# mhalushka/miRge3.0

Measured on NVIDIA B200. Metric: M reads/s trim+collapse+annotate, higher is better.
Workload: dtype u8/int32

## Files before the change

### mirge3.0_b200/csrc/adapter_search.cuh

```cuda
#pragma once
#ifdef ADAPTER_SEARCH_HOST
#include "host_shims.h"
#else
#include "common.cuh"
#endif

#define TRIM_THREADS 128
#define OB 64

struct DevAdapter {
  int where, m, min_overlap, indel_cost, wildcard_ref, k, effective_length;
  int link;
  uint64_t peq[5];
  int n_counts[MIRGE_MAX_ADAPTER_LEN + 1];
  int max_err[MIRGE_MAX_ADAPTER_LEN + 1];
  int acc[MIRGE_MAX_ADAPTER_LEN + 1];
  uint64_t a2;
  int wildcard_read;
  int general;
};
struct DevParams {
  int n_mods, kind[MIRGE_MAX_MODS], a[MIRGE_MAX_MODS], b[MIRGE_MAX_MODS], c[MIRGE_MAX_MODS];
  int n_adapters, times, min_len, umi_mode, umi5, umi3, qia_len, slots;
  int w_mis, w_indel;
  DevAdapter ad[MIRGE_MAX_ADAPTERS];
};
#ifdef ADAPTER_SEARCH_HOST
static DevParams c_p;
#else
__constant__ DevParams c_p;
#endif

static int trim_slots_of(const mirge_trim_params *p) {
  return (p->umi_mode != MIRGE_UMI_QIAGEN && p->count_mode == MIRGE_COUNT_HEAD) ? p->n_mods : 1;
}

#define FILL_FAIL(...)                  \
  do {                                  \
    snprintf(err, err_len, __VA_ARGS__); \
    return MIRGE_ERR_ARG;               \
  } while (0)

static int fill_dev_params(const mirge_trim_params *p, DevParams &d, int &maxm, int &fast_ok, char *err, size_t err_len) {
  if (p->n_mods < 0 || p->n_mods > MIRGE_MAX_MODS) FILL_FAIL("n_mods out of range");
  if (p->n_adapters < 0 || p->n_adapters > MIRGE_MAX_ADAPTERS) FILL_FAIL("n_adapters out of range");
  memset(&d, 0, sizeof(d));
  d.n_mods = p->n_mods;
  for (int i = 0; i < p->n_mods; ++i) {
    if (p->mod_kind[i] < MIRGE_MOD_NEXTSEQ || p->mod_kind[i] > MIRGE_MOD_CUT) FILL_FAIL("unknown modifier kind %d", p->mod_kind[i]);
    d.kind[i] = p->mod_kind[i];
    d.a[i] = p->mod_a[i];
    d.b[i] = p->mod_b[i];
    d.c[i] = p->mod_c[i];
  }
  d.n_adapters = p->n_adapters;
  d.times = p->times;
  d.min_len = p->min_len;
  d.umi_mode = p->umi_mode;
  d.umi5 = p->umi5;
  d.umi3 = p->umi3;
  d.qia_len = p->qia_adapter_len;
  d.slots = trim_slots_of(p);
  if (p->compat != MIRGE_COMPAT_CUTADAPT23 && p->compat != MIRGE_COMPAT_CUTADAPT4) FILL_FAIL("unknown cutadapt compat %d", p->compat);
  d.w_mis = p->compat == MIRGE_COMPAT_CUTADAPT4 ? -1 : 0;
  d.w_indel = p->compat == MIRGE_COMPAT_CUTADAPT4 ? -2 : 0;
  if (p->umi_mode < MIRGE_UMI_NONE || p->umi_mode > MIRGE_UMI_QIAGEN) FILL_FAIL("bad umi_mode");
  if (p->umi_mode != MIRGE_UMI_NONE && (p->umi5 < 0 || p->umi3 < 0)) FILL_FAIL("negative UMI length");
  if (p->umi_mode == MIRGE_UMI_QIAGEN && p->n_adapters < 1) FILL_FAIL("qiagen UMI mode needs an adapter");
  maxm = 0;
  fast_ok = p->n_adapters <= MIRGE_FAST_ADAPTERS;
  for (int a = 0; a < p->n_adapters; ++a) {
    const mirge_adapter *s = &p->adapters[a];
    if (s->m < 1 || s->m > MIRGE_MAX_ADAPTER_LEN) FILL_FAIL("adapter %d length %d unsupported", a, s->m);
    if (s->where < MIRGE_WHERE_BACK || s->where > MIRGE_WHERE_FRONT_NOT_INTERNAL) FILL_FAIL("adapter %d: unknown type", a);
    DevAdapter *o = &d.ad[a];
    o->where = s->where; o->m = s->m; o->min_overlap = s->min_overlap; o->indel_cost = s->indel_cost;
    o->wildcard_ref = s->wildcard_ref; o->k = s->k; o->effective_length = s->effective_length;
    o->link = s->link;
    o->wildcard_read = s->wildcard_read ? 1 : 0;
    o->general = (s->where > MIRGE_WHERE_FRONT || s->wildcard_read) ? 1 : 0;
    if (s->link != 0 && s->link != MIRGE_LINK_BACK_HALF) {
      const int b = (s->link & MIRGE_LINK_INDEX_MASK) - 1;
      if ((s->link & ~(MIRGE_LINK_INDEX_MASK | MIRGE_LINK_FRONT_OPTIONAL | MIRGE_LINK_BACK_OPTIONAL)) || !MIRGE_WHERE_IS_FRONT(s->where) ||
          b <= a || b >= p->n_adapters || MIRGE_WHERE_IS_FRONT(p->adapters[b].where) || p->adapters[b].link != MIRGE_LINK_BACK_HALF)
        FILL_FAIL("adapter %d: a linked pair is a 5' adapter followed by its 3' half", a);
      if (p->umi_mode == MIRGE_UMI_QIAGEN) FILL_FAIL("linked adapters are not supported with qiagen UMIs");
    }
    if (s->link != 0) fast_ok = 0;
    for (int c = 0; c < 4; ++c) {
      uint64_t bits = 0;
      for (int i = 0; i < s->m; ++i)
        if (s->mask[i] & (1 << c)) bits |= 1ull << i;
      o->peq[c] = bits;
    }
    o->peq[4] = 0;
    memcpy(o->n_counts, s->n_counts, sizeof(o->n_counts));
    memcpy(o->max_err, s->max_err, sizeof(o->max_err));
    for (int i = 0; i <= s->m; ++i) {
      const int eff = s->wildcard_ref ? i - s->n_counts[i] : i;
      o->acc[i] = (i >= s->min_overlap && i >= 1 && eff >= 0) ? s->max_err[eff] : -1;
    }
    o->a2 = 0;
    if (!s->wildcard_ref && s->m <= 32)
      for (int i = 0; i < s->m; ++i) {
        const uint64_t code = s->ascii[i] == 'A' ? 0 : s->ascii[i] == 'C' ? 1 : s->ascii[i] == 'G' ? 2 : 3;
        o->a2 |= code << (2 * i);
      }
    if (s->where != MIRGE_WHERE_BACK || s->wildcard_read || s->indel_cost != 1 || s->m > 32 || s->min_overlap < 1 || s->m + 2 * s->k + 3 > 48) fast_ok = 0;
    if (p->compat != MIRGE_COMPAT_CUTADAPT23) fast_ok = 0;
    if (s->m > maxm) maxm = s->m;
  }
  return MIRGE_OK;
}
#undef FILL_FAIL


struct Match { int rstart, rstop, matches, errors; };

#define MS 12
#define MM 0xFFF
__host__ __device__ __forceinline__ uint32_t iupac_set_upper(uint32_t c) {
  c &= 0xDFu;
  switch (c) {
    case 'A': return 1; case 'C': return 2; case 'G': return 4; case 'T': case 'U': return 8;
    case 'R': return 5; case 'Y': return 10; case 'S': return 6; case 'W': return 9; case 'K': return 12; case 'M': return 3;
    case 'B': return 14; case 'D': return 13; case 'H': return 11; case 'V': return 7; case 'N': return 15; default: return 0;
  }
}

template <int MAXM, bool GEN>
__device__ __noinline__ bool locate(const int a, const uint8_t *read, const int n, Match &out) {
  const DevAdapter &ad = c_p.ad[a];
  const int m = ad.m, ic = ad.indel_cost, k = ad.k;
  const bool back = ad.where == 0;
  const int w = ad.where;
  const bool start_in_ref = GEN ? (w == MIRGE_WHERE_FRONT || w == MIRGE_WHERE_FRONT_NOT_INTERNAL) : !back;
  const bool stop_in_ref = GEN ? (w == MIRGE_WHERE_BACK || w == MIRGE_WHERE_BACK_NOT_INTERNAL) : back;
  const bool start_in_query = GEN ? (w != MIRGE_WHERE_PREFIX && w != MIRGE_WHERE_FRONT_NOT_INTERNAL) : true;
  const bool stop_in_query = GEN ? (w != MIRGE_WHERE_SUFFIX && w != MIRGE_WHERE_BACK_NOT_INTERNAL) : true;
  const bool wild_read = GEN && ad.wildcard_read;
  const int max_n = (!GEN || start_in_query) ? n : min(n, m + k);
  const int min_n = (!GEN || stop_in_query) ? 0 : max(0, n - m - k);
  const int w_mis = c_p.w_mis, w_indel = c_p.w_indel;
  const int SB = w_indel ? 2048 : 0;
  const uint64_t p0 = ad.peq[0], p1 = ad.peq[1], p2 = ad.peq[2], p3 = ad.peq[3];
  int cost[MAXM + 1], om[MAXM + 1];
#pragma unroll
  for (int i = 0; i <= MAXM; ++i) {
    if (!GEN) {
      cost[i] = back ? i * ic : 0;
      om[i] = (((back ? 0 : -i) + OB) << MS) + SB + (back ? i * w_indel : 0);
    } else {
      int c, o;
      if (!start_in_ref && !start_in_query) { c = max(i, min_n) * ic; o = 0; }
      else if (start_in_ref && !start_in_query) { c = min_n * ic; o = min(0, min_n - i); }
      else if (!start_in_ref && start_in_query) { c = i * ic; o = max(0, min_n - i); }
      else { c = min(i, min_n) * ic; o = min_n - i; }
      cost[i] = c;
      om[i] = ((o + OB) << MS) + SB + (start_in_ref ? 0 : i * w_indel);
    }
  }
  int best_cost = m + n, best_om = (OB << MS) + (w_indel ? 0 : SB), best_ref_stop = m, best_query_stop = n;
  bool stopped = false;
  for (int j = min_n + 1; j <= max_n; ++j) {
    uint64_t eq;
    if (wild_read) {
      const uint32_t rs = iupac_set_upper(read[j - 1]);
      eq = ((rs & 1u) ? p0 : 0ull) | ((rs & 2u) ? p1 : 0ull) | ((rs & 4u) ? p2 : 0ull) | ((rs & 8u) ? p3 : 0ull);
    } else {
      const uint32_t rc = base_code_upper(read[j - 1]);
      eq = rc == 0 ? p0 : rc == 1 ? p1 : rc == 2 ? p2 : rc == 3 ? p3 : 0ull;
    }
    int dc = cost[0], dom = om[0];
    if (!GEN || start_in_query) om[0] = ((j + OB) << MS) + SB;
    else { cost[0] = j * ic; om[0] = (OB << MS) + SB + j * w_indel; }
    int cm = 0, omm = 0;
#pragma unroll
    for (int i = 1; i <= MAXM; ++i) {
      if (i <= m) {
        int c, o;
        if ((eq >> (i - 1)) & 1ull) {
          c = dc; o = dom + 1;
        } else {
          const int cd = dc + 1, cdel = cost[i] + ic, cins = cost[i - 1] + ic;
          if (cd <= cdel && cd <= cins) { c = cd; o = dom + w_mis; }
          else if (cins <= cdel) { c = cins; o = om[i - 1] + w_indel; }
          else { c = cdel; o = om[i] + w_indel; }
        }
        dc = cost[i]; dom = om[i];
        cost[i] = c; om[i] = o;
        if (i == m) { cm = c; omm = o; }
      }
    }
    if (cm <= k && (!GEN || stop_in_query)) {
      const int origin = (omm >> MS) - OB, mt = omm & MM;
      const int length = m + min(origin, 0);
      int eff = length;
      if (ad.wildcard_ref) eff = (length < m) ? length - (ad.n_counts[m] - ad.n_counts[m - length]) : ad.effective_length;
      const int bm = best_om & MM;
      if (length >= ad.min_overlap && cm <= ad.max_err[eff] && (mt > bm || (mt == bm && cm < best_cost))) {
        best_cost = cm; best_om = omm; best_ref_stop = m; best_query_stop = j;
        if (cm == 0 && mt - SB == m) { stopped = true; break; }
      }
    }
  }
  if (!stopped && (!GEN || max_n == n)) {
    const int first_i = stop_in_ref ? 0 : m;
#pragma unroll
    for (int i = 0; i <= MAXM; ++i) {
      if (i >= first_i && i <= m) {
        const int origin = (om[i] >> MS) - OB, mt = om[i] & MM, c = cost[i];
        const int length = i + min(origin, 0);
        int eff = length;
        if (ad.wildcard_ref) {
          if (length < m) { const int ref_start = origin < 0 ? -origin : 0; eff = length - (ad.n_counts[i] - ad.n_counts[ref_start]); }
          else eff = ad.effective_length;
        }
        const int bm = best_om & MM;
        if (length >= ad.min_overlap && eff >= 0 && c <= ad.max_err[eff] && (mt > bm || (mt == bm && c < best_cost))) {
          best_cost = c; best_om = om[i]; best_ref_stop = i; best_query_stop = n;
        }
      }
    }
  }
  (void)best_ref_stop;
  if (best_cost == m + n) return false;
  const int origin = (best_om >> MS) - OB;
  out.rstart = origin >= 0 ? origin : 0;
  out.rstop = best_query_stop;
  out.matches = (best_om & MM) - SB;
  out.errors = best_cost;
  return true;
}

__device__ __noinline__ bool find_literal(const int a, const uint8_t *read, const int n, Match &out) {
  const DevAdapter &ad = c_p.ad[a];
  const int m = ad.m;
  const uint64_t top = 1ull << (m - 1);
  uint64_t state = 0;
  for (int j = 0; j < n; ++j) {
    const uint32_t rc = base_code_upper(read[j]);
    state = ((state << 1) | 1ull) & (rc < 4u ? ad.peq[rc] : 0ull);
    if (state & top) {
      out.rstart = j + 1 - m;
      out.rstop = j + 1;
      out.matches = m;
      out.errors = 0;
      return true;
    }
  }
  return false;
}

template <int MAXM>
__device__ __forceinline__ bool locate_any(const int a, const uint8_t *read, const int n, Match &out) {
  const DevAdapter &ad = c_p.ad[a];
  if (!ad.general) return locate<MAXM, false>(a, read, n, out);
  if (ad.wildcard_read && !ad.wildcard_ref && ad.where <= MIRGE_WHERE_FRONT && find_literal(a, read, n, out)) return true;
  return locate<MAXM, true>(a, read, n, out);
}

#define RB 48

struct FastCtx {
  const uint32_t *s_eq;
  const uint32_t *ps;
  bool jump_ok;
  int rbase;
};

struct ByteRead {
  const uint8_t *p;
  __device__ __forceinline__ uint32_t eq(const uint32_t *eqt, int j) const { return eqt[p[j]]; }
  struct Cursor {
    const uint8_t *q;
    __device__ __forceinline__ uint32_t next(const uint32_t *eqt) { return eqt[*q++]; }
  };
  __device__ __forceinline__ Cursor cursor() const { return Cursor{p}; }
};
struct PackedRead {
  const uint32_t *ps;
  int base;
  __device__ __forceinline__ uint32_t eq(const uint32_t *eqt, int j) const {
    const int a = base + j;
    return eqt[(ps[(a >> 4) * TRIM_THREADS] >> (2 * (a & 15))) & 3u];
  }
  struct Cursor {
    const uint32_t *row;
    uint32_t w;
    int left;
    __device__ __forceinline__ uint32_t next(const uint32_t *eqt) {
      if (left == 0) {
        row += TRIM_THREADS;
        w = *row;
        left = 16;
      }
      const uint32_t code = w & 3u;
      w >>= 2;
      --left;
      return eqt[code];
    }
  };
  __device__ __forceinline__ Cursor cursor() const {
    const uint32_t *row = ps + (base >> 4) * TRIM_THREADS;
    const int sh = base & 15;
    return Cursor{row, *row >> (2 * sh), 16 - sh};
  }
};

struct ColBuf {
  uint32_t vp[RB], vn[RB];
  int j0;
};

__device__ __forceinline__ int cell_cost(uint32_t vp, uint32_t vn, int r) {
  const uint32_t mask = r >= 32 ? 0xFFFFFFFFu : ((1u << r) - 1u);
  return __popc(vp & mask) - __popc(vn & mask);
}

#define MYERS_STEP(eq, vp, vn, hp_out, hn_out)                    \
  {                                                               \
    const uint32_t xv_ = (eq) | (vn);                             \
    const uint32_t xh_ = ((((eq) & (vp)) + (vp)) ^ (vp)) | (eq);  \
    uint32_t hp_ = (vn) | ~(xh_ | (vp));                          \
    uint32_t hn_ = (vp) & xh_;                                    \
    hp_out = hp_;                                                 \
    hn_out = hn_;                                                 \
    hp_ <<= 1;                                                    \
    hn_ <<= 1;                                                    \
    (vp) = hn_ | ~(xv_ | hp_);                                    \
    (vn) = hp_ & xv_;                                             \
  }

template <class RV>
__device__ __noinline__ void recompute(const uint32_t *eqt, const RV read, int jc, int span, ColBuf &cb) {
  const int j0 = max(0, jc - span);
  uint32_t vp = 0xFFFFFFFFu, vn = 0u;
  cb.j0 = j0;
  cb.vp[0] = vp;
  cb.vn[0] = vn;
  int t = 1;
  for (int j = j0 + 1; j <= jc; ++j, ++t) {
    const uint32_t eq = read.eq(eqt, j - 1);
    uint32_t hp, hn;
    MYERS_STEP(eq, vp, vn, hp, hn)
    cb.vp[t] = vp;
    cb.vn[t] = vn;
  }
}

__device__ __forceinline__ uint64_t read_window(const uint32_t *ps, int a0) {
  const int wi = a0 >> 4, sh = 2 * (a0 & 15);
  const uint32_t w0 = ps[wi * TRIM_THREADS], w1 = ps[(wi + 1) * TRIM_THREADS], w2 = ps[(wi + 2) * TRIM_THREADS];
  const uint32_t lo = __funnelshift_r(w0, w1, sh), hi = __funnelshift_r(w1, w2, sh);
  return ((uint64_t)hi << 32) | lo;
}

template <class RV>
__device__ __noinline__ void traceback(const int a, const uint32_t *eqt, const RV read, const FastCtx &fc, const ColBuf &cb,
                                          int i, int j, int c, int &matches, int &origin) {
  const bool jump = fc.jump_ok && !c_p.ad[a].wildcard_ref;
  const uint64_t a2 = c_p.ad[a].a2;
  int r = i, col = j, cost = c, nonmatch = 0;
  while (r > 0 && cost > 0) {
    if (col == 0) {
      nonmatch += r;
      r = 0;
      break;
    }
    const int delta = col - r;
    if (jump && delta >= 0) {
      uint64_t x = a2 ^ read_window(fc.ps, fc.rbase + delta);
      x = (x | (x >> 1)) & 0x5555555555555555ull;
      if (r < 32) x &= (1ull << (2 * r)) - 1ull;
      if (x == 0) {
        col -= r;
        r = 0;
        break;
      }
      const int t = (64 - __clzll((long long)x) + 1) >> 1;
      col -= r - t;
      r = t;
    } else if ((read.eq(eqt, col - 1) >> (r - 1)) & 1u) {
      --r; --col;
      continue;
    }
    const int t0 = col - cb.j0;
    const uint32_t vp0 = cb.vp[t0], vn0 = cb.vn[t0], vp1 = cb.vp[t0 - 1], vn1 = cb.vn[t0 - 1];
    const int cd = cell_cost(vp1, vn1, r - 1) + 1, cdel = cell_cost(vp1, vn1, r) + 1, cins = cell_cost(vp0, vn0, r - 1) + 1;
    if (cd <= cdel && cd <= cins) { --r; --col; ++nonmatch; cost = cd - 1; }
    else if (cins <= cdel) { --r; ++nonmatch; cost = cins - 1; }
    else { --col; cost = cdel - 1; }
  }
  origin = col - r;
  matches = i - nonmatch;
}

__device__ __forceinline__ bool traceback_cost1(const int a, const FastCtx &fc, int i, int j, int &matches, int &origin) {
  const int delta = j - i;
  if (!fc.jump_ok || c_p.ad[a].wildcard_ref || delta < 0) return false;
  const uint64_t a2 = c_p.ad[a].a2;
  const uint64_t even = 0x5555555555555555ull;
  uint64_t x = a2 ^ read_window(fc.ps, fc.rbase + delta);
  x = (x | (x >> 1)) & even;
  if (i < 32) x &= (1ull << (2 * i)) - 1ull;
  if (x == 0) return false;
  const int t = (64 - __clzll((long long)x) + 1) >> 1;
  const uint64_t below = t - 1 >= 32 ? ~0ull : ((1ull << (2 * (t - 1))) - 1ull);
  if ((x & below) == 0) {
    matches = i - 1;
    origin = delta;
    return true;
  }
  uint64_t y = a2 ^ read_window(fc.ps, fc.rbase + delta + 1);
  y = (y | (y >> 1)) & even & below;
  if (y == 0) {
    matches = i - 1;
    origin = delta + 1;
    return true;
  }
  if (delta < 1) return false;
  const uint64_t upto = t >= 32 ? ~0ull : ((1ull << (2 * t)) - 1ull);
  uint64_t z = a2 ^ read_window(fc.ps, fc.rbase + delta - 1);
  z = (z | (z >> 1)) & even & upto;
  if (z != 0) return false;
  matches = i;
  origin = delta - 1;
  return true;
}

template <class RV>
__device__ __forceinline__ bool all_deletions_possible(const uint32_t *eqt, const RV read, int i, int j, int c) {
  const int o = j - i - c;
  return o >= 0 && (read.eq(eqt, o) & 1u);
}

#define MAY_WIN(u, c, idx) (!have || (u) > b_m || ((u) == b_m && ((c) < b_c || ((c) == b_c && (idx) < b_idx))))
#define TAKE_IF_BETTER(mt, c, org, idx)                                                      \
  if (!have || (mt) > b_m || ((mt) == b_m && ((c) < b_c || ((c) == b_c && (idx) < b_idx)))) { \
    have = true; b_m = (mt); b_c = (c); b_o = (org); b_idx = (idx);                          \
  }
#define Q_COL(v) ((int)((v)&0xFFFFu))
#define Q_COST(v) ((int)(((v) >> 16) & 0xFFu))
#define Q_UB(v, m) ((((v) >> 24) & 1u) ? (m) : (m)-1)
#define Q_CHAIN(v) ((int)((v) >> 25))
#define INS_MASK(eq, vp, hn) (~(eq) & (vp) & ((hn) << 1))
#define CHAIN_LEN(ins, i) (__clz((int)~((ins) << (32 - (i)))))

template <bool DEFER, class RV>
__device__ __forceinline__ int locate_fast(const int a, const RV read, const int n, const FastCtx &fc, Match &out) {
  const unsigned lanes = __activemask();
  const DevAdapter &ad = c_p.ad[a];
  const int m = ad.m;
  const int span = m + 2 * ad.k + 2;
  const uint32_t *eqt = fc.s_eq + a * 256;
  const uint32_t top = 1u << (m - 1);
  const int acc_m = ad.acc[m];
  uint32_t vp = 0xFFFFFFFFu, vn = 0u, eq = 0;
  int score = m;
  bool have = false;
  int b_m = 0, b_c = 0, b_o = 0, b_idx = 0;
  bool stopped = false;
  ColBuf cb;
  uint32_t q0 = 0, q1 = 0, q2 = 0, q3 = 0;
  bool pend = false, pend_ins = false, need_slow = false;
  uint32_t pend_v = 0;

#define FLUSH_QUEUE()                                                                            \
  for (int it_ = 0; it_ < 4; ++it_) {                                                            \
    uint32_t v_ = 0;                                                                             \
    int which_ = -1;                                                                             \
    if (q0 && (!v_ || Q_COST(q0) < Q_COST(v_))) { v_ = q0; which_ = 0; }                         \
    if (q1 && (!v_ || Q_COST(q1) < Q_COST(v_))) { v_ = q1; which_ = 1; }                         \
    if (q2 && (!v_ || Q_COST(q2) < Q_COST(v_))) { v_ = q2; which_ = 2; }                         \
    if (q3 && (!v_ || Q_COST(q3) < Q_COST(v_))) { v_ = q3; which_ = 3; }                         \
    if (which_ < 0) break;                                                                       \
    if (which_ == 0) q0 = 0; else if (which_ == 1) q1 = 0; else if (which_ == 2) q2 = 0; else q3 = 0; \
    const int jc_ = Q_COL(v_), cc_ = Q_COST(v_), t_ = Q_CHAIN(v_);                               \
    const int ir_ = m - t_, cr_ = cc_ - t_;           \
    int ub_ = t_ ? ir_ : Q_UB(v_, m);                                                            \
    if (!t_ && ub_ == m && !all_deletions_possible(eqt, read, m, jc_, cc_)) ub_ = m - 1;        \
    if (MAY_WIN(ub_, cc_, jc_)) {                                                                \
      int mt_, org_;                                                                             \
      if (cr_ == 0) {                                                                            \
        mt_ = ir_; org_ = jc_ - ir_;                                                             \
      } else if (!(cr_ == 1 && traceback_cost1(a, fc, ir_, jc_, mt_, org_))) {                   \
        if (DEFER) { need_slow = true; break; }                                                  \
        recompute(eqt, read, jc_, span, cb);                                                     \
        traceback(a, eqt, read, fc, cb, ir_, jc_, cr_, mt_, org_);                               \
      }                                                                                          \
      TAKE_IF_BETTER(mt_, cc_, org_, jc_)                                                        \
    }                                                                                            \
  }

  uint32_t hp = 0, hn = 0;
  auto cur = read.cursor();
  for (int j = 1; j <= n; ++j) {
    eq = cur.next(eqt);
    MYERS_STEP(eq, vp, vn, hp, hn)
    score += (hp & top) ? 1 : 0;
    score -= (hn & top) ? 1 : 0;
    if (pend) {
      if (!(pend_ins && (eq & top))) {
        if (!q0) q0 = pend_v;
        else if (!q1) q1 = pend_v;
        else if (!q2) q2 = pend_v;
        else if (!q3) q3 = pend_v;
        else {
          FLUSH_QUEUE()
          if (DEFER && need_slow) break;
          q0 = pend_v;
        }
      }
      pend = false;
    }
    if (score <= acc_m && j < n) {
      if (score == 0) {
        have = true; b_m = m; b_c = 0; b_o = j - m; b_idx = j;
        stopped = true;
        break;
      }
      bool is_del = false, is_ins = false;
      const bool is_match = (eq & top) != 0u;
      if (!is_match) {
        const uint32_t hps = hp << 1, hns = hn << 1;
        const bool mis = (((vp & ~hps & ~hns) | (~vp & ~vn & hps)) & top) != 0u;
        if (!mis) {
          if (vp & top) is_ins = true;
          else is_del = true;
        }
      }
      if (!is_del) {
        pend = true;
        pend_ins = is_ins;
        const uint32_t chain = is_ins ? 1u + (uint32_t)CHAIN_LEN(INS_MASK(eq, vp, hn), m - 1) : 0u;
        pend_v = (uint32_t)j | ((uint32_t)score << 16) | (is_match ? (1u << 24) : 0u) | (chain << 25);
      }
    }
  }
  __syncwarp(lanes);
  const unsigned scan_lanes = __ballot_sync(lanes, !stopped && !need_slow);
  if (!stopped && !need_slow) {
    uint32_t rowmask = 0, rowub = 0;
    const uint32_t hps = hp << 1, hns = hn << 1;
    const uint32_t ins = n >= 1 ? INS_MASK(eq, vp, hn) : 0u;
    const uint32_t mis = n >= 1 ? (~eq & ((vp & ~hps & ~hns) | (~vp & ~vn & hps))) : 0u;
    int c = 0;
    for (int i = 1; i <= m; ++i) {
      const uint32_t bit = 1u << (i - 1);
      c += (int)((vp >> (i - 1)) & 1u) - (int)((vn >> (i - 1)) & 1u);
      if (c > ad.acc[i]) continue;
      if (c == 0) {
        const int idx = (i == m) ? n : n + 1 + i;
        TAKE_IF_BETTER(i, 0, n - i, idx)
      } else if (ins & bit) {
        const int t = CHAIN_LEN(ins, i);
        if (ad.acc[i - t] >= c - t) continue;
        rowmask |= bit;
      } else {
        rowmask |= bit;
        if ((eq & bit) || !(mis & bit)) rowub |= bit;
      }
    }
    __syncwarp(scan_lanes);
    FLUSH_QUEUE()
    bool have_cols = false;
    while (rowmask) {
      const int i = 32 - __clz(rowmask);
      const uint32_t bit = 1u << (i - 1);
      rowmask &= ~bit;
      const int ci = cell_cost(vp, vn, i);
      const int idx = (i == m) ? n : n + 1 + i;
      const int t = (ins & bit) ? CHAIN_LEN(ins, i) : 0;
      const int ir = i - t, cr = ci - t;
      int ub = t ? ir : ((rowub & bit) ? i : i - 1);
      if (!t && ub == i && !all_deletions_possible(eqt, read, i, n, ci)) ub = i - 1;
      if (MAY_WIN(ub, ci, idx)) {
        int mt, org;
        if (cr == 0) {
          mt = ir;
          org = n - ir;
        } else if (!(cr == 1 && traceback_cost1(a, fc, ir, n, mt, org))) {
          if (DEFER) { need_slow = true; break; }
          if (!have_cols) {
            recompute(eqt, read, n, span, cb);
            have_cols = true;
          }
          traceback(a, eqt, read, fc, cb, ir, n, cr, mt, org);
        }
        TAKE_IF_BETTER(mt, ci, org, idx)
      }
    }
  }
  if (DEFER && need_slow) return 2;
  if (!have) return 0;
  out.rstart = b_o;
  out.rstop = b_idx <= n ? b_idx : n;
  out.matches = b_m;
  out.errors = b_c;
  return 1;
}


__device__ __forceinline__ int nextseq_trim_index(const uint8_t *seq, const uint8_t *qual, int len, int cutoff, int base) {
  int s = 0, max_qual = 0, max_i = len;
  for (int i = len - 1; i >= 0; --i) {
    int q = (int)qual[i] - base;
    if (seq[i] == 'G') q = cutoff - 1;
    s += cutoff - q;
    if (s < 0) break;
    if (s > max_qual) { max_qual = s; max_i = i; }
  }
  return max_i;
}

__device__ __forceinline__ void quality_trim_index(const uint8_t *qual, int len, int q5, int q3, int base, int &start, int &stop) {
  int s = 0, max_qual = 0;
  start = 0; stop = len;
  for (int i = 0; i < len; ++i) {
    s += q5 - ((int)qual[i] - base);
    if (s < 0) break;
    if (s > max_qual) { max_qual = s; start = i + 1; }
  }
  max_qual = 0; s = 0;
  for (int i = len - 1; i >= 0; --i) {
    s += q3 - ((int)qual[i] - base);
    if (s < 0) break;
    if (s > max_qual) { max_qual = s; stop = i; }
  }
  if (start >= stop) { start = 0; stop = 0; }
}


template <int MAXM, bool FAST, bool DEFER>
__device__ __noinline__ int best_match(const uint8_t *read, int n, Match &best, const FastCtx &fc) {
  int which = -1;
  for (int a = 0; a < c_p.n_adapters; ++a) {
    Match mt;
    const int link = c_p.ad[a].link;
    if (link == MIRGE_LINK_BACK_HALF) continue;
    if (FAST) {
      const int rc = locate_fast<DEFER>(a, ByteRead{read}, n, fc, mt);
      if (rc == 2) return -2;
      if (rc == 0) continue;
    } else if (link != 0) {
      Match f, b;
      const bool have_f = locate_any<MAXM>(a, read, n, f);
      if (!have_f && !(link & MIRGE_LINK_FRONT_OPTIONAL)) continue;
      const int rest = have_f ? f.rstop : 0;
      const bool have_b = locate_any<MAXM>((link & MIRGE_LINK_INDEX_MASK) - 1, read + rest, n - rest, b);
      if (!have_b && (!(link & MIRGE_LINK_BACK_OPTIONAL) || !have_f)) continue;
      mt.rstart = rest;
      mt.rstop = have_b ? rest + b.rstart : n;
      mt.matches = (have_f ? f.matches : 0) + (have_b ? b.matches : 0);
      mt.errors = (have_f ? f.errors : 0) + (have_b ? b.errors : 0);
    } else if (!locate_any<MAXM>(a, read, n, mt)) continue;
    if (which < 0 || mt.matches > best.matches || (mt.matches == best.matches && mt.errors < best.errors)) {
      best = mt;
      which = a;
    }
  }
  return which;
}

template <int MAXM, bool FAST, bool DEFER>
__device__ __noinline__ bool apply_mod(int mi, const uint8_t *seq, const uint8_t *qual, int &start, int &stop, FastCtx &fc) {
  const int len = stop - start;
  switch (c_p.kind[mi]) {
    case MIRGE_MOD_NEXTSEQ:
      stop = start + nextseq_trim_index(seq + start, qual + start, len, c_p.a[mi], c_p.b[mi]);
      break;
    case MIRGE_MOD_QUALITY: {
      int s, e;
      quality_trim_index(qual + start, len, c_p.a[mi], c_p.b[mi], c_p.c[mi], s, e);
      stop = start + e;
      start = start + s;
      break;
    }
    case MIRGE_MOD_ADAPTER:
      for (int t = 0; t < c_p.times; ++t) {
        Match mt;
        fc.rbase = start;
        const int a = best_match<MAXM, FAST, DEFER>(seq + start, stop - start, mt, fc);
        if (a == -2) return true;
        if (a < 0) break;
        if (c_p.ad[a].link != 0) { stop = start + mt.rstop; start = start + mt.rstart; }
        else if (!MIRGE_WHERE_IS_FRONT(c_p.ad[a].where)) stop = start + mt.rstart;
        else start = start + mt.rstop;
      }
      break;
    case MIRGE_MOD_NEND:
      while (start < stop && seq[start] == 'N') ++start;
      while (stop > start && seq[stop - 1] == 'N') --stop;
      break;
    case MIRGE_MOD_CUT: {
      const int c = c_p.a[mi];
      if (c > 0) start += min(c, len);
      else stop = start + max(len + c, 0);
      break;
    }
    default: break;
  }
  return false;
}
```

### mirge3.0_b200/csrc/trim.cu

```cuda
#include "common.cuh"
#include "adapter_search.cuh"

extern "C" int mirge_trim_slots(const mirge_ctx *ctx) {
  if (!ctx || !ctx->params_set) return MIRGE_ERR_ARG;
  return trim_slots_of(&ctx->params);
}

extern "C" int mirge_set_trim_params(mirge_ctx *ctx, const mirge_trim_params *p) {
  if (!ctx || !p) return MIRGE_ERR_ARG;
  DevParams d;
  int maxm = 0, fast_ok = 1;
  const int rc = fill_dev_params(p, d, maxm, fast_ok, ctx->err, sizeof(ctx->err));
  if (rc != MIRGE_OK) return rc;
  MIRGE_CUDA(ctx, cudaSetDevice(ctx->device));
  MIRGE_CUDA(ctx, cudaMemcpyToSymbol(c_p, &d, sizeof(d)));
  ctx->params = *p;
  ctx->params_set = 1;
  ctx->max_adapter_len = maxm;
  ctx->fast_ok = fast_ok;
  int split_ok = fast_ok && p->umi_mode != MIRGE_UMI_QIAGEN, seen_ad = 0;
  for (int i = 0; i < p->n_mods; ++i) {
    if (p->mod_kind[i] == MIRGE_MOD_ADAPTER) seen_ad = 1;
    else if (seen_ad && (p->mod_kind[i] == MIRGE_MOD_NEXTSEQ || p->mod_kind[i] == MIRGE_MOD_QUALITY)) split_ok = 0;
  }
  ctx->split_ok = split_ok && seen_ad;
  return MIRGE_OK;
}

__device__ __forceinline__ void apply_plain_mod(int mi, const uint8_t *seq, const uint8_t *qual, int &start, int &stop) {
  const int len = stop - start;
  const int kind = c_p.kind[mi];
  if (kind == MIRGE_MOD_NEXTSEQ) {
    stop = start + nextseq_trim_index(seq + start, qual + start, len, c_p.a[mi], c_p.b[mi]);
  } else if (kind == MIRGE_MOD_QUALITY) {
    int s, e;
    quality_trim_index(qual + start, len, c_p.a[mi], c_p.b[mi], c_p.c[mi], s, e);
    stop = start + e;
    start = start + s;
  } else if (kind == MIRGE_MOD_NEND) {
    while (start < stop && seq[start] == 'N') ++start;
    while (stop > start && seq[stop - 1] == 'N') --stop;
  } else if (kind == MIRGE_MOD_CUT) {
    const int c = c_p.a[mi];
    if (c > 0) start += min(c, len);
    else stop = start + max(len + c, 0);
  }
}

__device__ __forceinline__ int find_sub(const uint8_t *s, int n, const uint8_t *t, int tl, int from) {
  for (int p = from; p + tl <= n; ++p) {
    int j = 0;
    while (j < tl && s[p + j] == t[j]) ++j;
    if (j == tl) return p;
  }
  return -1;
}

__device__ __forceinline__ uint32_t key_byte(const uint8_t *seq, int start, int l1, int us, int p) {
  return p < l1 ? seq[start + p] : seq[us + p - l1];
}

#define MAX_PACK_WORDS 10
#define PS_ROWS_OF(pw) ((pw) + 3)
__shared__ int s_pack_words;
#define PACK_WORDS s_pack_words
#define PS_ROWS PS_ROWS_OF(s_pack_words)

struct DpEntry {
  uint32_t r;
  uint32_t se;
  uint32_t sl;
  uint32_t pad;
};

struct SlowRec {
  uint32_t r, x, y, z, w, nxt, pad0, pad1;
};
struct SlowSink {
  uint32_t *r_list;
  SlowRec *recs;
  uint64_t cap;
};

__device__ __forceinline__ int first_adapter_mod() {
  int mi_ad = c_p.n_mods;
#pragma unroll 1
  for (int i = c_p.n_mods - 1; i >= 0; --i)
    if (c_p.kind[i] == MIRGE_MOD_ADAPTER) mi_ad = i;
  return mi_ad;
}

__device__ __forceinline__ int exact_find(const uint32_t *ps, uint64_t a2, int m, int start, int stop) {
  const int last = stop - m;
  if (last < start) return -1;
  const uint32_t a_lo = (uint32_t)a2, a_hi = (uint32_t)(a2 >> 32);
  const uint32_t lo_mask = m >= 16 ? 0xFFFFFFFFu : ((1u << (2 * m)) - 1u);
  const uint32_t hi_mask = m <= 16 ? 0u : (m >= 32 ? 0xFFFFFFFFu : ((1u << (2 * (m - 16))) - 1u));
  int wb = start >> 4;
  uint32_t x0 = ps[wb * TRIM_THREADS], x1 = ps[(wb + 1) * TRIM_THREADS], x2 = ps[(wb + 2) * TRIM_THREADS];
#pragma unroll 1
  for (; 16 * wb <= last; ++wb) {
#pragma unroll
    for (int s = 0; s < 16; ++s) {
      const uint32_t lo = s ? __funnelshift_r(x0, x1, 2 * s) : x0;
      if (((lo ^ a_lo) & lo_mask) == 0u) {
        const uint32_t hi = s ? __funnelshift_r(x1, x2, 2 * s) : x1;
        const int p = 16 * wb + s;
        if (((hi ^ a_hi) & hi_mask) == 0u && p >= start && p <= last) return p;
      }
    }
    x0 = x1;
    x1 = x2;
    x2 = (wb + 3 < PS_ROWS) ? ps[(wb + 3) * TRIM_THREADS] : 0u;
  }
  return -1;
}

struct InsList {
  uint2 *off;
  uint64_t cap;
};
#define WORD_BITS 36
#define WORD_MASK ((1ull << WORD_BITS) - 1ull)
#define MAX_LIST_ITEMS (1ull << (64 - WORD_BITS))

__shared__ unsigned int s_stats[2];
__device__ __forceinline__ void init_stats(int pack_words) {
  if (threadIdx.x < 2) s_stats[threadIdx.x] = 0;
  if (threadIdx.x == 0) s_pack_words = pack_words;
}
__device__ __forceinline__ void flush_stats(unsigned long long *ctrl) {
  __syncthreads();
  if (threadIdx.x == 0) {
    if (s_stats[0]) atomicAdd(ctrl + 1, (unsigned long long)s_stats[0]);
    if (s_stats[1]) atomicAdd(ctrl + 4, (unsigned long long)s_stats[1]);
  }
}

template <bool FAST, int PASS>
__device__ __forceinline__ void emit_record(const bool valid, const uint64_t r, const int E, const int slot_lo, const int slot_hi,
                                            const uint8_t *seq, const bool fast_emit, const int *w_start, const int *w_stop,
                                            const int *w_us, const int *w_ue, uint32_t *w_words, const bool to_slow,
                                            ushort4 *__restrict__ win, uint32_t *__restrict__ key_off, uint32_t *__restrict__ keys,
                                            uint64_t keys_cap, unsigned long long *__restrict__ ctrl, const SlowSink ss, const uint4 ls,
                                            const uint32_t nxt, const uint32_t *ps_mine, const InsList il) {
  const int lane = threadIdx.x & 31;
  uint32_t my_words = 0, my_kept = 0, my_alg = 0, same_as_prev = 0, my_items = 0;
  if (valid) {
#pragma unroll 1
    for (int s = slot_lo; s < slot_hi; ++s) {
      if (!w_words[s]) continue;
      ++my_kept;
      if (s > slot_lo && w_words[s - 1] && w_start[s] == w_start[s - 1] && w_stop[s] == w_stop[s - 1] && w_us[s] == w_us[s - 1] &&
          w_ue[s] == w_ue[s - 1]) {
        w_words[s] = w_words[s - 1];
        my_alg += w_words[s];
        same_as_prev |= 1u << s;
        continue;
      }
      if (FAST && fast_emit) {
        w_words[s] = 1u + ((uint32_t)(w_stop[s] - w_start[s] + 15) >> 4);
      } else {
        const int l1 = w_stop[s] - w_start[s], len = l1 + (w_ue[s] - w_us[s]);
        uint32_t nexc = 0;
        for (int p = 0; p < len; ++p) nexc += base_code_exact(key_byte(seq, w_start[s], l1, w_us[s], p)) == 4u;
        w_words[s] = 1u + ((uint32_t)(len + 15) >> 4) + nexc;
      }
      my_words += w_words[s];
      my_alg += w_words[s];
      ++my_items;
    }
  }
  uint32_t inc = my_words | (my_items << 24);
#pragma unroll
  for (int d = 1; d < 32; d <<= 1) {
    const uint32_t t = __shfl_up_sync(0xffffffffu, inc, d);
    if (lane >= d) inc += t;
  }
  const uint32_t both_total = __shfl_sync(0xffffffffu, inc, 31);
  const uint32_t warp_total = both_total & 0xFFFFFFu, warp_items = both_total >> 24;
  const uint32_t item_before = (inc >> 24) - my_items;
  inc &= 0xFFFFFFu;
  const uint32_t kept_warp = __reduce_add_sync(0xffffffffu, my_kept);
  const uint32_t alg_warp = __reduce_add_sync(0xffffffffu, my_alg);
  unsigned long long both = 0;
  if (lane == 0) {
    if (both_total) both = atomicAdd(ctrl + 0, ((unsigned long long)warp_items << WORD_BITS) | (unsigned long long)warp_total);
    if (kept_warp) atomicAdd(&s_stats[0], kept_warp);
    if (alg_warp) atomicAdd(&s_stats[1], alg_warp);
  }
  both = __shfl_sync(0xffffffffu, both, 0);
  const unsigned long long warp_base = both & WORD_MASK, item_base = both >> WORD_BITS;
  const bool overflow = warp_base + warp_total > keys_cap || warp_base + warp_total > 0xFFFFFFF0ull;
  if (overflow && lane == 0 && warp_total) atomicOr(ctrl + 2, 2ull);
  if (PASS == 1) {
    const unsigned sm_ = __ballot_sync(0xffffffffu, to_slow);
    if (sm_) {
      unsigned long long base = 0;
      if (lane == __ffs(sm_) - 1) base = atomicAdd(ctrl + 5, (unsigned long long)__popc(sm_));
      base = __shfl_sync(0xffffffffu, base, __ffs(sm_) - 1);
      if (to_slow) {
        const unsigned long long at = base + __popc(sm_ & ((1u << lane) - 1u));
        if (!ss.recs) {
          ss.r_list[at] = (uint32_t)r;
        } else if (at < ss.cap) {
          SlowRec sr;
          sr.r = (uint32_t)r; sr.x = ls.x; sr.y = ls.y; sr.z = ls.z; sr.w = ls.w; sr.nxt = nxt; sr.pad0 = sr.pad1 = 0;
          *(uint4 *)&ss.recs[at] = *(const uint4 *)&sr;
          *((uint4 *)&ss.recs[at] + 1) = *((const uint4 *)&sr + 1);
        } else {
          atomicOr(ctrl + 2, 8ull);
        }
      }
    }
  }
  if (!valid) return;
  uint32_t off = (uint32_t)warp_base + inc - my_words;
  uint64_t item = item_base + item_before;
#pragma unroll 1
  for (int s = slot_lo; s < slot_hi; ++s) {
    const uint64_t e = r * (uint64_t)E + s;
    if (win) win[e] = make_ushort4((unsigned short)w_start[s], (unsigned short)w_stop[s], (unsigned short)w_us[s], (unsigned short)w_ue[s]);
    if (!w_words[s] || overflow) {
      if (key_off) key_off[e] = 0xFFFFFFFFu;
      continue;
    }
    if ((same_as_prev >> s) & 1u) {
      if (key_off) key_off[e] = off - w_words[s];
      continue;
    }
    if (key_off) key_off[e] = off;
    if (il.off && item < il.cap) {
      const uint32_t run = (uint32_t)__ffs((int)(~(same_as_prev >> (s + 1)) | (1u << (slot_hi - s - 1))));
      il.off[item] = make_uint2(off, run);
      ++item;
    }
    const int l1 = w_stop[s] - w_start[s], len = l1 + (w_ue[s] - w_us[s]);
    const uint32_t npay = (uint32_t)(len + 15) >> 4;
    uint32_t *k = keys + off;
    if (FAST && fast_emit) {
      k[0] = (uint32_t)len;
      const int wi = w_start[s] >> 4;
      const uint32_t bs = 2u * (uint32_t)(w_start[s] & 15);
      uint32_t lo = ps_mine[wi * TRIM_THREADS];
#pragma unroll 1
      for (uint32_t w = 0; w < npay; ++w) {
        const uint32_t hi = ps_mine[(wi + w + 1) * TRIM_THREADS];
        uint32_t v = __funnelshift_r(lo, hi, bs);
        lo = hi;
        const int rem = len - 16 * (int)w;
        if (rem < 16) v &= (1u << (2 * rem)) - 1u;
        k[1 + w] = v;
      }
    } else {
      const uint32_t nexc = w_words[s] - 1u - npay;
      k[0] = (uint32_t)len | (nexc << 16);
      uint32_t word = 0, xi = 0;
      for (int p = 0; p < len; ++p) {
        const uint32_t ch = key_byte(seq, w_start[s], l1, w_us[s], p);
        const uint32_t code = base_code_exact(ch);
        if (code == 4u) k[1 + npay + xi++] = ((uint32_t)p << 8) | ch;
        else word |= code << (2 * (p & 15));
        if ((p & 15) == 15) { k[1 + (p >> 4)] = word; word = 0; }
      }
      if (len & 15) k[1 + (len >> 4)] = word;
    }
    off += w_words[s];
  }
}

#define RECORD_SLOT(mi_)                                                                         \
  if (!qia && (E != 1 || (mi_) == n_mods - 1)) {                                                 \
    const int slot_ = (E == 1) ? 0 : (mi_);                                                      \
    int ln_ = stop - start;                                                                      \
    if (c_p.umi_mode == MIRGE_UMI_FLANKS) ln_ = max(ln_ - c_p.umi5 - c_p.umi3, 0);               \
    w_start[slot_] = start; w_stop[slot_] = stop; w_words[slot_] = ln_ >= c_p.min_len;           \
  }

struct SplitOut {
  DpEntry *entries;
  uint32_t *pk;
  uint64_t cap;
};

template <int MAXM, bool FAST, int PASS, bool SPLIT>
__device__ __forceinline__ void process_record(const bool valid, const uint64_t r, const uint8_t *B, uint64_t nbytes,
                                               const uint32_t *__restrict__ line_start, ushort4 *__restrict__ win,
                                               uint32_t *__restrict__ key_off, uint32_t *__restrict__ keys, uint64_t keys_cap,
                                               unsigned long long *__restrict__ ctrl, const SlowSink ss, FastCtx &fc,
                                               uint32_t *ps_mine, const SplitOut so, const uint4 ls, const uint32_t nxt,
                                               const InsList il) {
  const int lane = threadIdx.x & 31;
  bool is_slow = false;
  const int E = c_p.slots;
  const int n_mods = c_p.n_mods;
  const bool qia = c_p.umi_mode == MIRGE_UMI_QIAGEN;
  int w_start[MIRGE_MAX_MODS], w_stop[MIRGE_MAX_MODS], w_us[MIRGE_MAX_MODS], w_ue[MIRGE_MAX_MODS];
  uint32_t w_words[MIRGE_MAX_MODS];
#pragma unroll 1
  for (int s = 0; s < E; ++s) { w_start[s] = w_stop[s] = w_us[s] = w_ue[s] = 0; w_words[s] = 0; }
  const uint8_t *seq = nullptr, *qual = nullptr;
  uint32_t seq_off = 0;
  bool fast_emit = FAST, good = false;
  int sl = 0, start = 0, stop = 0;
  if (valid) {
    sl = (int)(ls.z - 1 - ls.y);
    int ql = (int)(nxt - 1 - ls.w);
    if (sl > 0 && B[ls.y + sl - 1] == '\r') --sl;
    if (ql > 0 && B[ls.w + ql - 1] == '\r') --ql;
    const bool bad = B[ls.x] != '@' || B[ls.z] != '+' || sl != ql || sl > MIRGE_MAX_READ_LEN;
    if (bad) {
      atomicOr(ctrl + 2, (sl > MIRGE_MAX_READ_LEN && sl == ql) ? 4ull : 1ull);
      atomicMax(ctrl + 3, ~(unsigned long long)r);
    } else {
      good = true;
      seq_off = ls.y;
      seq = B + ls.y;
      qual = B + ls.w;
      stop = sl;
    }
  }
  const unsigned good_lanes = __ballot_sync(0xffffffffu, good);
  if (good && FAST) {
    fast_emit = sl <= 16 * PACK_WORDS;
    if (PASS == 2 && (uint64_t)seq_off + 16 * ((sl + 15) >> 4) + 8 > nbytes) fast_emit = false;
    if (fast_emit) {
      const uint32_t *ap = (const uint32_t *)((uintptr_t)seq & ~(uintptr_t)3);
      const uint32_t bs = ((uint32_t)(uintptr_t)seq & 3u) * 8u;
      const int nwords = (sl + 15) >> 4;
      uint32_t anyexc = 0, prev = ap[0];
      int k = 1;
#pragma unroll 1
      for (int w = 0; w < nwords; ++w) {
        uint32_t word = 0;
#pragma unroll
        for (int q4 = 0; q4 < 4; ++q4) {
          const uint32_t nx = ap[k++];
          const uint32_t quad = __funnelshift_r(prev, nx, bs);
          prev = nx;
          const int nb = sl - (16 * w + 4 * q4);
          uint32_t codes = ((quad >> 1) ^ (quad >> 2)) & 0x03030303u;
          uint32_t sel = codes | (codes >> 4);
          sel = (sel & 0xFFu) | ((sel >> 8) & 0xFF00u);
          uint32_t diff = __byte_perm(0x54474341u, 0u, sel) ^ quad;
          if (nb < 4) {
            const uint32_t tm = nb <= 0 ? 0u : (0xFFFFFFFFu >> (8 * (4 - nb)));
            codes &= tm;
            diff &= tm;
          }
          anyexc |= diff;
          word |= ((codes * 0x01041040u) >> 24) << (8 * q4);
        }
        ps_mine[w * TRIM_THREADS] = word;
      }
#pragma unroll 1
      for (int w = nwords; w < PS_ROWS; ++w) ps_mine[w * TRIM_THREADS] = 0;
      if (anyexc) fast_emit = false;
    }
    fc.jump_ok = fast_emit;
  }

#define RUN_MODS(from_, to_)                                                                     \
  _Pragma("unroll 1") for (int mi = (from_); mi < (to_); ++mi) {                                 \
    if (!is_slow) is_slow = apply_mod<MAXM, FAST, PASS == 1>(mi, seq, qual, start, stop, fc);    \
    __syncwarp(good_lanes);                                                                      \
    RECORD_SLOT(mi)                                                                              \
  }

  int slot_lo = 0, slot_hi = E;
  bool to_slow = false;
  if constexpr (!SPLIT) {
    if (good) { RUN_MODS(0, n_mods) }
  } else {
    const int mi_ad = first_adapter_mod();
    if (good) {
      _Pragma("unroll 1") for (int mi = 0; mi < mi_ad; ++mi) {
        apply_plain_mod(mi, seq, qual, start, stop);
        __syncwarp(good_lanes);
        RECORD_SLOT(mi)
      }
    }
    bool to_dp = false, resolved = false;
    if (good && mi_ad < n_mods) {
      const DevAdapter &ad0 = c_p.ad[0];
      const bool exact_ok = c_p.n_adapters == 1 && c_p.times == 1 && !ad0.wildcard_ref && ad0.acc[ad0.m] >= 0;
      int p = -1;
      if (fc.jump_ok && exact_ok) p = exact_find(ps_mine, ad0.a2, ad0.m, start, stop);
      __syncwarp(good_lanes);
      if (!fc.jump_ok) {
        is_slow = true;
      } else if (p >= 0) {
        stop = p;
        resolved = true;
      } else {
        to_dp = true;
      }
      if (resolved) { RECORD_SLOT(mi_ad) }
    }
    if (good) {
      _Pragma("unroll 1") for (int mi = mi_ad + 1; mi < n_mods; ++mi) {
        if (resolved && !is_slow) {
          const int kind = c_p.kind[mi];
          if (kind == MIRGE_MOD_NEND) {
            while (start < stop && seq[start] == 'N') ++start;
            while (stop > start && seq[stop - 1] == 'N') --stop;
          } else if (kind == MIRGE_MOD_CUT) {
            const int c = c_p.a[mi], len = stop - start;
            if (c > 0) start += min(c, len);
            else stop = start + max(len + c, 0);
          } else {
            is_slow = true;
          }
        }
        __syncwarp(good_lanes);
        if (resolved) { RECORD_SLOT(mi) }
      }
    }
    const unsigned dm = __ballot_sync(0xffffffffu, to_dp);
    if (dm) {
      const int leader = __ffs(dm) - 1;
      unsigned long long base = 0;
      if (lane == leader) base = atomicAdd(ctrl + 6, (unsigned long long)__popc(dm));
      base = __shfl_sync(0xffffffffu, base, leader);
      if (to_dp) {
        const uint64_t e = base + __popc(dm & ((1u << lane) - 1u));
        DpEntry de;
        de.r = (uint32_t)r; de.se = (uint32_t)start | ((uint32_t)stop << 16); de.sl = (uint32_t)sl; de.pad = 0;
        *(uint4 *)(so.entries + e) = *(const uint4 *)&de;
        const int nwords = (sl + 15) >> 4;
#pragma unroll 1
        for (int w = 0; w < nwords; ++w) so.pk[(uint64_t)w * so.cap + e] = ps_mine[w * TRIM_THREADS];
      }
    }
    if (to_dp) slot_hi = (E == 1) ? 0 : mi_ad;
  }
#undef RUN_MODS

  if (good) {
    if (qia) {
      const int tl = stop - start, U = c_p.umi3;
      int us = 0, ue = 0;
      if (tl > 0) {
        const int first = find_sub(seq, sl, seq + start, tl, 0);
        const int after = first + tl;
        const int nx = find_sub(seq, sl, seq + start, tl, after);
        int seg_end = nx < 0 ? sl : nx;
        seg_end = min(seg_end, after + c_p.qia_len + U);
        ue = seg_end;
        us = (U != 0) ? max(seg_end - U, after) : after;
      }
      w_start[0] = start; w_stop[0] = stop; w_us[0] = us; w_ue[0] = ue;
      w_words[0] = (tl >= c_p.min_len) ? 1u : 0u;
      if (ue > us) fast_emit = false;
    }
    if (PASS == 1 && is_slow) {
      slot_hi = slot_lo;
      to_slow = true;
    }
  }
  emit_record<FAST, PASS>(valid, r, E, slot_lo, slot_hi, seq, fast_emit, w_start, w_stop, w_us, w_ue, w_words, to_slow, win, key_off,
                          keys, keys_cap, ctrl, ss, ls, nxt, ps_mine, il);
}

__device__ __noinline__ bool find_lines(const uint8_t *fq, uint64_t n, uint4 &ls, uint32_t &nxt, bool virtual_nl) {
  uint32_t found[4];
  int k = 0;
  for (uint64_t p = ls.x; p < n && k < 4; ++p)
    if (fq[p] == '\n') found[k++] = (uint32_t)p + 1u;
  if (k == 3 && virtual_nl && n > found[2]) found[k++] = (uint32_t)n + 1u;
  if (k < 4) return false;
  ls.y = found[0]; ls.z = found[1]; ls.w = found[2];
  nxt = found[3];
  return true;
}

template <int MAXM, bool FAST, int PASS, bool SPLIT>
__global__ void __launch_bounds__(TRIM_THREADS, (FAST && PASS == 1) ? 7 : 1)
trim_kernel(const uint8_t *__restrict__ fq, uint64_t nbytes, const uint32_t *__restrict__ line_start, uint64_t n_records,
            ushort4 *__restrict__ win, uint32_t *__restrict__ key_off, uint32_t *__restrict__ keys, uint64_t keys_cap,
            unsigned long long *__restrict__ ctrl, uint32_t smem_bytes, uint32_t *__restrict__ d_slow, const SplitOut so,
            const InsList il, const int pack_words, const SlowRec *__restrict__ slow_recs, const uint32_t n_cap) {
  extern __shared__ uint4 smem4[];
  uint8_t *sbuf = (uint8_t *)smem4;
  const int tid = threadIdx.x;
  FastCtx fc;
  fc.s_eq = nullptr; fc.ps = nullptr; fc.jump_ok = false; fc.rbase = 0;
  uint32_t *ps_mine = nullptr;
  init_stats(pack_words);
  if (FAST) {
    uint32_t *eq = (uint32_t *)(sbuf + smem_bytes);
    for (int e = tid; e < c_p.n_adapters * 256; e += TRIM_THREADS) {
      const uint32_t code = base_code_upper((uint32_t)(e & 255));
      eq[e] = code < 4u ? (uint32_t)c_p.ad[e >> 8].peq[code] : 0u;
    }
    fc.s_eq = eq;
    ps_mine = eq + c_p.n_adapters * 256 + tid;
    fc.ps = ps_mine;
  }
  const SlowSink ss{d_slow, nullptr, 0};
  if (PASS == 2) {
    __syncthreads();
    unsigned long long n_slow = ctrl[5];
    if (slow_recs && n_slow > n_cap) n_slow = n_cap;
    const uint64_t first = (uint64_t)blockIdx.x * TRIM_THREADS + (tid & ~31);
    for (uint64_t base = first; base < n_slow; base += (uint64_t)gridDim.x * TRIM_THREADS) {
      const uint64_t idx = base + (tid & 31);
      bool valid = idx < n_slow;
      uint64_t r = 0;
      fc.jump_ok = false;
      uint4 ls = make_uint4(0, 0, 0, 0);
      uint32_t nxt = 0;
      if (valid && slow_recs) {
        const uint4 a = *(const uint4 *)&slow_recs[idx], b = *((const uint4 *)&slow_recs[idx] + 1);
        r = a.x;
        ls = make_uint4(a.y, a.z, a.w, b.x);
        nxt = b.y;
        if (ls.y == 0) valid = find_lines(fq, nbytes, ls, nxt, b.z != 0);
        if (valid && r >= n_cap) {
          atomicOr(ctrl + 2, 16ull);
          valid = false;
        }
        if (valid && line_start) {
          uint32_t *lo = const_cast<uint32_t *>(line_start);
          lo[4 * r] = ls.x; lo[4 * r + 1] = ls.y; lo[4 * r + 2] = ls.z; lo[4 * r + 3] = ls.w; lo[4 * r + 4] = nxt;
        }
      } else if (valid) {
        r = d_slow[idx];
        ls = *(const uint4 *)(line_start + 4 * r);
        nxt = line_start[4 * r + 4];
      }
      process_record<MAXM, FAST, 2, false>(valid, r, fq, nbytes, line_start, win, key_off, keys, keys_cap, ctrl,
                                           ss, fc, ps_mine, so, ls, nxt, il);
      __syncwarp();
    }
    flush_stats(ctrl);
    return;
  }
  const uint64_t r0 = (uint64_t)blockIdx.x * TRIM_THREADS;
  const uint64_t r = r0 + tid;
  const bool valid = r < n_records;
  const uint64_t r_end = min(r0 + (uint64_t)TRIM_THREADS, n_records);
  const uint32_t span_lo = line_start[4 * r0];
  const uint64_t span_hi = min((uint64_t)line_start[4 * r_end], nbytes);
  const uint32_t alo = span_lo & ~15u;
  const bool staged = (span_hi - alo) <= smem_bytes;
  if (FAST && !staged) {
    if (PASS == 1) {
      const unsigned vm = __ballot_sync(0xffffffffu, valid);
      if (vm) {
        const int lane = tid & 31;
        unsigned long long base = 0;
        if (lane == __ffs(vm) - 1) base = atomicAdd(ctrl + 5, (unsigned long long)__popc(vm));
        base = __shfl_sync(0xffffffffu, base, __ffs(vm) - 1);
        if (valid) d_slow[base + __popc(vm & ((1u << lane) - 1u))] = (uint32_t)r;
      }
      return;
    }
    if (tid == 0) atomicOr(ctrl + 2, 8ull);
    return;
  }
  if (staged) {
    for (uint64_t o = (uint64_t)tid * 16; alo + o < span_hi; o += TRIM_THREADS * 16) {
      const uint64_t g = alo + o;
      if (g + 16 <= nbytes) {
        cp_async_16(sbuf + o, fq + g);
      } else {
        for (int b = 0; b < 16 && g + b < nbytes; ++b) sbuf[o + b] = fq[g + b];
      }
    }
    cp_async_wait_all();
  }
  __syncthreads();
  uint4 ls = make_uint4(0, 0, 0, 0);
  uint32_t nxt = 0;
  if (valid) { ls = *(const uint4 *)(line_start + 4 * r); nxt = line_start[4 * r + 4]; }
  const uint8_t *B = staged ? (const uint8_t *)(sbuf - alo) : fq;
  process_record<MAXM, FAST, PASS, SPLIT>(valid, r, B, nbytes, line_start, win, key_off, keys, keys_cap, ctrl, ss, fc, ps_mine, so, ls, nxt, il);
  flush_stats(ctrl);
}

#ifndef DT_TILE
#define DT_TILE 16384
#endif
#define DT_OVH 2048
#define DT_LOAD (DT_TILE + DT_OVH)
#define DT_WORDS (DT_LOAD / 32)
#ifndef DT_NBUF
#define DT_NBUF 2
#endif
#ifndef DT_GROUPS
#define DT_GROUPS 1
#endif
#define DT_CWARPS (DT_GROUPS * TRIM_THREADS / 32)
#define DT_THREADS (32 + DT_GROUPS * TRIM_THREADS)
#define DT_FLAG_AGG (1ull << 62)
#define DT_FLAG_INC (2ull << 62)
#define DT_VAL_MASK ((1ull << 62) - 1ull)
static_assert(DT_TILE % 1024 == 0 && DT_LOAD % 1024 == 0, "the producer scans 1 KB per step");

struct TileMeta {
  unsigned long long before;
  unsigned long long tile_lo;
  uint32_t n_rec;
  uint32_t j0;
  uint32_t nload;
  uint32_t first;
  uint32_t n_nl;
  uint32_t at_end;
};

struct DigestTilesArgs {
  const uint8_t *fq;
  unsigned long long n;
  uint32_t skew;
  uint32_t is_final;
  unsigned long long n_tiles;
  unsigned long long *tile_state;
  uint32_t *line_start;
  uint32_t n_cap;
  ushort4 *win;
  uint32_t *key_off;
  uint32_t *keys;
  unsigned long long keys_cap;
  unsigned long long *ctrl;
  SlowSink ss;
  SplitOut so;
  InsList il;
  int pack_words;
};

__device__ __forceinline__ uint32_t nl_position(const uint32_t *mask, const uint16_t *pref, uint32_t j, uint32_t &w_out) {
  uint32_t lo = 0, hi = DT_WORDS;
  while (hi - lo > 1) {
    const uint32_t mid = (lo + hi) >> 1;
    if (pref[mid] <= j) lo = mid; else hi = mid;
  }
  uint32_t m = mask[lo];
  for (uint32_t k = j - pref[lo]; k; --k) m &= m - 1;
  w_out = lo;
  return 32u * lo + (uint32_t)(__ffs((int)m) - 1);
}
__device__ __forceinline__ uint32_t nl_next(const uint32_t *mask, uint32_t p, uint32_t &w) {
  const uint32_t bit = p & 31u;
  uint32_t m = bit == 31u ? 0u : (mask[w] & (0xFFFFFFFEu << bit));
  while (m == 0u) {
    if (++w >= DT_WORDS) return 0xFFFFFFFFu;
    m = mask[w];
  }
  return 32u * w + (uint32_t)(__ffs((int)m) - 1);
}

__global__ void __launch_bounds__(DT_THREADS, 3) digest_tiles_kernel(const __grid_constant__ DigestTilesArgs A) {
  extern __shared__ uint4 smem4[];
  __shared__ uint64_t bar_full[DT_NBUF], bar_ready[DT_NBUF], bar_empty[DT_NBUF];
  __shared__ TileMeta s_meta[DT_NBUF];
  __shared__ uint32_t s_next[DT_NBUF];
  uint8_t *bufs = (uint8_t *)smem4;
  uint32_t *masks = (uint32_t *)(bufs + DT_NBUF * DT_LOAD);
  uint16_t *prefs = (uint16_t *)(masks + DT_NBUF * DT_WORDS);
  uint32_t *eq = (uint32_t *)(prefs + DT_NBUF * (DT_WORDS + 2));
  uint32_t *ps_base = eq + c_p.n_adapters * 256;
  const int tid = threadIdx.x, lane = tid & 31, warp = tid >> 5;
  unsigned long long *ctrl = A.ctrl;
  init_stats(A.pack_words);
  for (int e = tid; e < c_p.n_adapters * 256; e += DT_THREADS) {
    const uint32_t code = base_code_upper((uint32_t)(e & 255));
    eq[e] = code < 4u ? (uint32_t)c_p.ad[e >> 8].peq[code] : 0u;
  }
  if (tid == 0) {
    for (int b = 0; b < DT_NBUF; ++b) {
      mbar_init(&bar_full[b], 1);
      mbar_init(&bar_ready[b], 1);
      mbar_init(&bar_empty[b], DT_CWARPS);
    }
    asm volatile("fence.mbarrier_init.release.cluster;" ::: "memory");
  }
  __syncthreads();
  const bool virtual_nl = A.is_final && A.n > A.skew && A.fq[A.n - 1] != '\n';

  if (warp == 0) {
    for (uint32_t it = 0;; ++it) {
      const int b = it % DT_NBUF;
      const uint32_t par = (it / DT_NBUF) & 1u;
      if (it >= DT_NBUF) mbar_wait(&bar_empty[b], par ^ 1u);
      unsigned long long t = 0;
      if (lane == 0) t = atomicAdd(ctrl + 11, 1ull);
      t = __shfl_sync(0xffffffffu, t, 0);
      TileMeta &M = s_meta[b];
      if (t >= A.n_tiles) {
        if (lane == 0) {
          M.n_rec = 0xFFFFFFFFu;
          mbar_arrive(&bar_ready[b]);
        }
        break;
      }
      const unsigned long long tile_lo = t * DT_TILE;
      const uint32_t nload = (uint32_t)min((unsigned long long)DT_LOAD, A.n - tile_lo);
      const uint32_t bulk = nload & ~15u;
      uint8_t *buf = bufs + b * DT_LOAD;
      if (lane == 0) {
        if (bulk) {
          mbar_arrive_expect_tx(&bar_full[b], bulk);
          bulk_load(buf, A.fq + tile_lo, bulk, &bar_full[b]);
        } else {
          mbar_arrive(&bar_full[b]);
        }
      }
      if ((uint32_t)lane < nload - bulk) buf[bulk + lane] = A.fq[tile_lo + bulk + lane];
      __syncwarp();
      mbar_wait(&bar_full[b], par);
      uint32_t *mk = masks + b * DT_WORDS;
      uint16_t *pf = prefs + b * (DT_WORDS + 2);
      const uint32_t vpos = (virtual_nl && A.n - tile_lo < DT_LOAD) ? (uint32_t)(A.n - tile_lo) : 0xFFFFFFFFu;
      uint32_t running = 0, tile_total = 0;
#pragma unroll 1
      for (uint32_t w0 = 0; w0 < DT_WORDS; w0 += 32) {
        const uint32_t w = w0 + lane, pos = 32u * w;
        uint32_t m = 0;
        if (pos < nload) {
          const uint4 a = *(const uint4 *)(buf + pos), c = *(const uint4 *)(buf + pos + 16);
          const uint32_t ww[8] = {a.x, a.y, a.z, a.w, c.x, c.y, c.z, c.w};
          m = newline_mask(ww);
          if (pos + 32 > nload) m &= (1u << (nload - pos)) - 1u;
          if (t == 0 && w == 0) m &= ~((1u << A.skew) - 1u);
        }
        if (vpos >= pos && vpos < pos + 32) m |= 1u << (vpos - pos);
        mk[w] = m;
        const uint32_t c = __popc(m);
        uint32_t inc = c;
#pragma unroll
        for (int d = 1; d < 32; d <<= 1) {
          const uint32_t x = __shfl_up_sync(0xffffffffu, inc, d);
          if (lane >= d) inc += x;
        }
        pf[w] = (uint16_t)(running + inc - c);
        running += __shfl_sync(0xffffffffu, inc, 31);
        if (w0 + 32 == DT_TILE / 32) tile_total = running;
      }
      if (lane == 0) pf[DT_WORDS] = (uint16_t)running;
      __syncwarp();
      unsigned long long before = 0;
      if (lane == 0) {
        volatile unsigned long long *st = A.tile_state;
        if (t == 0) {
          st[0] = DT_FLAG_INC | (unsigned long long)tile_total;
        } else {
          st[t] = DT_FLAG_AGG | (unsigned long long)tile_total;
          __threadfence();
          unsigned long long p = t;
          while (true) {
            --p;
            unsigned long long v;
            while (((v = st[p]) >> 62) == 0ull) {}
            before += v & DT_VAL_MASK;
            if ((v >> 62) == 2ull) break;
          }
          st[t] = DT_FLAG_INC | (before + tile_total);
        }
        __threadfence();
        if (tile_total) atomicAdd(ctrl + 9, (unsigned long long)tile_total);
      }
      before = __shfl_sync(0xffffffffu, before, 0);
      const uint32_t j0 = (3u - (uint32_t)(before & 3ull)) & 3u;
      const uint32_t n_rec = tile_total > j0 ? (tile_total - j0 + 3u) / 4u : 0u;
      if (lane == 0) {
        if (n_rec) {
          uint32_t wq;
          const uint32_t pe = nl_position(mk, pf, j0 + 4u * (n_rec - 1u), wq);
          atomicMax(ctrl + 10, tile_lo + pe + 1ull);
        }
        M.before = before; M.tile_lo = tile_lo; M.n_rec = n_rec; M.j0 = j0; M.nload = nload; M.first = t == 0 ? 1u : 0u;
        M.n_nl = running; M.at_end = tile_lo + nload >= A.n ? 1u : 0u;
        s_next[b] = 0;
        __threadfence_block();
        mbar_arrive(&bar_ready[b]);
      }
      __syncwarp();
    }
  } else {
    const int ctid = tid - 32, group = ctid / TRIM_THREADS;
    uint32_t *ps_mine = ps_base + group * PS_ROWS_OF(A.pack_words) * TRIM_THREADS + (ctid & (TRIM_THREADS - 1));
    FastCtx fc;
    fc.s_eq = eq; fc.ps = ps_mine; fc.jump_ok = false; fc.rbase = 0;
    for (uint32_t it = 0;; ++it) {
      const int b = it % DT_NBUF;
      const uint32_t par = (it / DT_NBUF) & 1u;
      mbar_wait(&bar_ready[b], par);
      const TileMeta M = s_meta[b];
      if (M.n_rec == 0xFFFFFFFFu) break;
      const uint32_t *mk = masks + b * DT_WORDS;
      const uint16_t *pf = prefs + b * (DT_WORDS + 2);
      const uint8_t *B = bufs + b * DT_LOAD - M.tile_lo;
      const uint32_t total = M.n_rec + M.first;
      while (true) {
        uint32_t c = 0;
        if (lane == 0) c = atomicAdd(&s_next[b], 32u);
        c = __shfl_sync(0xffffffffu, c, 0);
        if (c >= total) break;
        const uint32_t q = c + lane;
        bool valid = q < total, far = false;
        uint64_t r = 0;
        uint4 ls = make_uint4(0, 0, 0, 0);
        uint32_t nxt = 0;
        if (valid) {
          uint32_t p, w = 0;
          if (M.first && q == 0) {
            ls.x = A.skew;
            p = 0xFFFFFFFFu;
          } else {
            const uint32_t j = M.j0 + 4u * (q - M.first);
            p = nl_position(mk, pf, j, w);
            ls.x = (uint32_t)M.tile_lo + p + 1u;
            r = (M.before + j + 1ull) >> 2;
          }
          uint32_t e[4];
          bool all = true;
#pragma unroll
          for (int k = 0; k < 4; ++k) {
            if (all) {
              if (p == 0xFFFFFFFFu && k == 0) {
                p = M.n_nl ? nl_position(mk, pf, 0u, w) : 0xFFFFFFFFu;
              } else {
                p = nl_next(mk, p, w);
              }
              all = p != 0xFFFFFFFFu;
              e[k] = (uint32_t)M.tile_lo + p + 1u;
            }
          }
          if (all) {
            ls.y = e[0]; ls.z = e[1]; ls.w = e[2];
            nxt = e[3];
          } else if (M.at_end) {
            valid = false;
          } else {
            far = true;
            valid = false;
          }
          if ((valid || far) && r >= A.n_cap) {
            atomicOr(ctrl + 2, 16ull);
            valid = far = false;
          }
          if (valid && A.line_start) {
            *(uint4 *)(A.line_start + 4 * r) = ls;
            A.line_start[4 * r + 4] = nxt;
          }
        }
        const unsigned fm = __ballot_sync(0xffffffffu, far);
        if (fm) {
          unsigned long long fb = 0;
          if (lane == __ffs(fm) - 1) fb = atomicAdd(ctrl + 5, (unsigned long long)__popc(fm));
          fb = __shfl_sync(0xffffffffu, fb, __ffs(fm) - 1);
          if (far) {
            const unsigned long long at = fb + __popc(fm & ((1u << lane) - 1u));
            if (at < A.ss.cap) {
              SlowRec sr;
              sr.r = (uint32_t)r; sr.x = ls.x; sr.y = 0; sr.z = 0; sr.w = 0; sr.nxt = 0; sr.pad0 = virtual_nl ? 1u : 0u; sr.pad1 = 0;
              *(uint4 *)&A.ss.recs[at] = *(const uint4 *)&sr;
              *((uint4 *)&A.ss.recs[at] + 1) = *((const uint4 *)&sr + 1);
            } else {
              atomicOr(ctrl + 2, 8ull);
            }
          }
        }
        process_record<32, true, 1, true>(valid, r, B, A.n, nullptr, A.win, A.key_off, A.keys, A.keys_cap, ctrl, A.ss, fc, ps_mine,
                                          A.so, ls, nxt, A.il);
        __syncwarp();
      }
      __syncwarp();
      if (lane == 0) mbar_arrive(&bar_empty[b]);
    }
  }
  flush_stats(ctrl);
}

template <bool FIRST>
__global__ void __launch_bounds__(TRIM_THREADS, FIRST ? 7 : 4)
trim_dp_kernel(const DpEntry *__restrict__ entries, const uint32_t *__restrict__ pk, uint64_t cap, uint32_t *__restrict__ redo,
               ushort4 *__restrict__ win, uint32_t *__restrict__ key_off, uint32_t *__restrict__ keys, uint64_t keys_cap,
               unsigned long long *__restrict__ ctrl, const InsList il, const int pack_words) {
  extern __shared__ uint4 smem4[];
  uint32_t *eq = (uint32_t *)smem4;
  uint32_t *ps_base = eq + c_p.n_adapters * 256;
  DpEntry *s_ent = (DpEntry *)(ps_base + PS_ROWS_OF(pack_words) * TRIM_THREADS);
  uint32_t *s_hist = (uint32_t *)(s_ent + TRIM_THREADS);
  uint16_t *s_order = (uint16_t *)(s_hist + TRIM_THREADS);
  const int tid = threadIdx.x, lane = tid & 31;
  const unsigned long long n_items = FIRST ? ctrl[6] : ctrl[7];
  const uint64_t base = (uint64_t)blockIdx.x * TRIM_THREADS;
  if (base >= n_items) return;
  init_stats(pack_words);
  for (int e = tid; e < c_p.n_adapters * 4; e += TRIM_THREADS) eq[(e >> 2) * 256 + (e & 3)] = (uint32_t)c_p.ad[e >> 2].peq[e & 3];
  const int n_here = (int)min((unsigned long long)TRIM_THREADS, n_items - base);
  uint32_t my_e = 0;
  int bin = TRIM_THREADS - 1;
  if (tid < n_here) {
    my_e = FIRST ? (uint32_t)(base + tid) : redo[base + tid];
    const uint4 v = *(const uint4 *)(entries + my_e);
    DpEntry de = *(const DpEntry *)&v;
    de.pad = my_e;
    s_ent[tid] = de;
    const int wl = (int)(de.se >> 16) - (int)(de.se & 0xFFFFu);
    bin = TRIM_THREADS - 1 - min(wl, TRIM_THREADS - 1);
  }
  s_hist[tid] = 0;
  __syncthreads();
  if (tid < n_here) atomicAdd(&s_hist[bin], 1u);
  __syncthreads();
  if (tid < 32) {
    uint32_t h[TRIM_THREADS / 32], sum = 0;
#pragma unroll
    for (int q = 0; q < TRIM_THREADS / 32; ++q) { h[q] = s_hist[(TRIM_THREADS / 32) * tid + q]; sum += h[q]; }
    uint32_t incl = sum;
#pragma unroll
    for (int d = 1; d < 32; d <<= 1) {
      const uint32_t x = __shfl_up_sync(0xffffffffu, incl, d);
      if (lane >= d) incl += x;
    }
    uint32_t run = incl - sum;
#pragma unroll
    for (int q = 0; q < TRIM_THREADS / 32; ++q) { s_hist[(TRIM_THREADS / 32) * tid + q] = run; run += h[q]; }
  }
  __syncthreads();
  if (tid < n_here) s_order[atomicAdd(&s_hist[bin], 1u)] = (uint16_t)tid;
  __syncthreads();
  const bool valid = tid < n_here;
  const int E = c_p.slots, n_mods = c_p.n_mods;
  const bool qia = false;
  int w_start[MIRGE_MAX_MODS], w_stop[MIRGE_MAX_MODS], w_us[MIRGE_MAX_MODS], w_ue[MIRGE_MAX_MODS];
  uint32_t w_words[MIRGE_MAX_MODS];
#pragma unroll 1
  for (int s = 0; s < E; ++s) { w_start[s] = w_stop[s] = w_us[s] = w_ue[s] = 0; w_words[s] = 0; }
  uint32_t *ps_mine = ps_base + tid;
  const int mi_ad = first_adapter_mod();
  uint64_t r = 0;
  bool need_redo = false;
  int slot_lo = (E == 1) ? 0 : mi_ad, slot_hi = E;
  uint32_t ent_id = 0;
  if (valid) {
    const DpEntry de = s_ent[s_order[tid]];
    r = de.r;
    ent_id = de.pad;
    int start = (int)(de.se & 0xFFFFu), stop = (int)(de.se >> 16);
    const int nwords = ((int)de.sl + 15) >> 4;
#pragma unroll 1
    for (int w = 0; w < PS_ROWS_OF(pack_words); ++w) {
      if (w < nwords) cp_async_4(ps_mine + w * TRIM_THREADS, pk + (uint64_t)w * cap + ent_id);
      else ps_mine[w * TRIM_THREADS] = 0u;
    }
    cp_async_wait_all();
    FastCtx fc;
    fc.s_eq = eq; fc.ps = ps_mine; fc.jump_ok = true; fc.rbase = 0;
#pragma unroll 1
    for (int mi = mi_ad; mi < n_mods && !need_redo; ++mi) {
      const int kind = c_p.kind[mi];
      if (kind == MIRGE_MOD_ADAPTER) {
#pragma unroll 1
        for (int t = 0; t < c_p.times; ++t) {
          fc.rbase = start;
          const PackedRead rv{ps_mine, start};
          const int n = stop - start;
          Match best;
          int which = -1;
#pragma unroll 1
          for (int a = 0; a < c_p.n_adapters; ++a) {
            Match mt;
            const int rc = locate_fast<FIRST>(a, rv, n, fc, mt);
            if (rc == 2) { need_redo = true; break; }
            if (rc == 0) continue;
            if (which < 0 || mt.matches > best.matches || (mt.matches == best.matches && mt.errors < best.errors)) { best = mt; which = a; }
          }
          if (need_redo || which < 0) break;
          stop = start + best.rstart;
        }
      } else if (kind == MIRGE_MOD_CUT) {
        const int c = c_p.a[mi], len = stop - start;
        if (c > 0) start += min(c, len);
        else stop = start + max(len + c, 0);
      }
      if (!need_redo) { RECORD_SLOT(mi) }
    }
  }
  if (FIRST) {
    const unsigned rm = __ballot_sync(0xffffffffu, need_redo);
    if (rm) {
      const int leader = __ffs(rm) - 1;
      unsigned long long b2 = 0;
      if (lane == leader) b2 = atomicAdd(ctrl + 7, (unsigned long long)__popc(rm));
      b2 = __shfl_sync(0xffffffffu, b2, leader);
      if (need_redo) redo[b2 + __popc(rm & ((1u << lane) - 1u))] = ent_id;
    }
    if (need_redo) slot_hi = slot_lo;
  }
  emit_record<true, 0>(valid, r, E, slot_lo, slot_hi, nullptr, true, w_start, w_stop, w_us, w_ue, w_words, false, win, key_off, keys, keys_cap,
                       ctrl, SlowSink{nullptr, nullptr, 0}, make_uint4(0, 0, 0, 0), 0u, ps_mine, il);
  flush_stats(ctrl);
}

static uint64_t align16(uint64_t x) { return (x + 15) & ~15ull; }
extern "C" uint64_t mirge_trim_scratch_bytes(uint64_t n_records) {
  const uint64_t n = n_records ? n_records : 1;
  return 2 * align16(4 * n) + align16(sizeof(DpEntry) * n) + align16(4ull * MAX_PACK_WORDS * n) + 64;
}

extern "C" int mirge_trim(mirge_ctx *ctx, const uint8_t *d_fastq, uint64_t nbytes, const uint32_t *d_line_start, uint64_t n_records,
                          uint16_t *d_win, uint32_t *d_key_off, uint32_t *d_keys, uint64_t keys_capacity_words,
                          uint64_t *d_trim_ctrl, void *d_scratch, uint64_t *d_ins, uint64_t ins_capacity, void *stream_) {
  if (!ctx) return MIRGE_ERR_ARG;
  if (!ctx->params_set) MIRGE_FAIL(ctx, MIRGE_ERR_ARG, "trim: mirge_set_trim_params has not been called");
  if (n_records == 0) return MIRGE_OK;
  if (!d_fastq || !d_line_start || !d_keys || !d_trim_ctrl) MIRGE_FAIL(ctx, MIRGE_ERR_ARG, "trim: null buffer");
  if (!d_win != !d_key_off) MIRGE_FAIL(ctx, MIRGE_ERR_ARG, "trim: d_win and d_key_off go together");
  if (!d_key_off && !d_ins) MIRGE_FAIL(ctx, MIRGE_ERR_ARG, "trim: neither per-slot outputs nor an insert list requested");
  if (d_ins && (ins_capacity == 0 || ((uintptr_t)d_ins & 7))) MIRGE_FAIL(ctx, MIRGE_ERR_ARG, "trim: bad insert list");
  if (n_records * (uint64_t)trim_slots_of(&ctx->params) >= MAX_LIST_ITEMS)
    MIRGE_FAIL(ctx, MIRGE_ERR_ARG, "trim: more than 2^28 emission slots in one batch (use smaller batches)");
  if (((uintptr_t)d_line_start & 15) || ((uintptr_t)d_win & 7) || ((uintptr_t)d_scratch & 15))
    MIRGE_FAIL(ctx, MIRGE_ERR_ARG, "trim: misaligned buffer");
  const InsList il{(uint2 *)d_ins, d_ins ? ins_capacity : 0};
  if (n_records >= 0x80000000ull) MIRGE_FAIL(ctx, MIRGE_ERR_ARG, "trim: more than 2^31 records in one batch");
  {
    const uint32_t skew = (uint32_t)((uintptr_t)d_fastq & 15);
    d_fastq -= skew;
    nbytes += skew;
  }
  cudaStream_t stream = (cudaStream_t)stream_;
  MIRGE_CUDA(ctx, cudaSetDevice(ctx->device));
  const uint64_t avg = (nbytes + n_records - 1) / n_records;
  const bool fast = ctx->fast_ok && ctx->trim_mode != 1;
  const bool split = fast && ctx->split_ok && ctx->trim_mode == 0;
  uint64_t want = fast ? avg * TRIM_THREADS * 33 / 32 + 512 : avg * TRIM_THREADS * 5 / 4 + 64;
  want = (want + 255) & ~255ull;
  if (want < 4096) want = 4096;
  if (want > 96 * 1024) want = 96 * 1024;
  const uint32_t smem = (uint32_t)want;
  const unsigned grid = (unsigned)((n_records + TRIM_THREADS - 1) / TRIM_THREADS);
  unsigned long long *ctrl = (unsigned long long *)d_trim_ctrl;
  ushort4 *win = (ushort4 *)d_win;
  SplitOut so;
  so.entries = nullptr; so.pk = nullptr; so.cap = 0;
  if (fast) {
    if (!d_scratch) MIRGE_FAIL(ctx, MIRGE_ERR_ARG, "trim: scratch of mirge_trim_scratch_bytes(n_records) bytes is required");
    uint8_t *sc = (uint8_t *)d_scratch;
    uint32_t *d_slow = (uint32_t *)sc;
    uint32_t *d_redo = (uint32_t *)(sc + align16(4 * n_records));
    so.entries = (DpEntry *)(sc + 2 * align16(4 * n_records));
    so.pk = (uint32_t *)(sc + 2 * align16(4 * n_records) + align16(sizeof(DpEntry) * n_records));
    so.cap = n_records;
    const int pack_words = avg <= 2 * 112 + 40 ? 8 : MAX_PACK_WORDS;
    const size_t extra = (size_t)ctx->params.n_adapters * 1024 + (size_t)PS_ROWS_OF(pack_words) * TRIM_THREADS * 4;
    if (split) {
      MIRGE_CUDA(ctx, cudaFuncSetAttribute(trim_kernel<32, true, 1, true>, cudaFuncAttributeMaxDynamicSharedMemorySize, 200 * 1024));
      trim_kernel<32, true, 1, true><<<grid, TRIM_THREADS, smem + extra, stream>>>(d_fastq, nbytes, d_line_start, n_records, win, d_key_off,
                                                                                 d_keys, keys_capacity_words, ctrl, smem, d_slow, so, il, pack_words, nullptr, 0u);
      MIRGE_LAUNCH_CHECK(ctx, "trim_kernel(stage 1)");
      const size_t dp_smem = extra + (size_t)TRIM_THREADS * (sizeof(DpEntry) + 4 + 2);
      trim_dp_kernel<true><<<grid, TRIM_THREADS, dp_smem, stream>>>(so.entries, so.pk, so.cap, d_redo, win, d_key_off, d_keys,
                                                                    keys_capacity_words, ctrl, il, pack_words);
      MIRGE_LAUNCH_CHECK(ctx, "trim_dp_kernel(stage 2)");
      trim_dp_kernel<false><<<grid, TRIM_THREADS, dp_smem, stream>>>(so.entries, so.pk, so.cap, d_redo, win, d_key_off, d_keys,
                                                                     keys_capacity_words, ctrl, il, pack_words);
      MIRGE_LAUNCH_CHECK(ctx, "trim_dp_kernel(stage 3)");
    } else {
      MIRGE_CUDA(ctx, cudaFuncSetAttribute(trim_kernel<32, true, 1, false>, cudaFuncAttributeMaxDynamicSharedMemorySize, 200 * 1024));
      trim_kernel<32, true, 1, false><<<grid, TRIM_THREADS, smem + extra, stream>>>(d_fastq, nbytes, d_line_start, n_records, win,
                                                                                  d_key_off, d_keys, keys_capacity_words, ctrl, smem,
                                                                                  d_slow, so, il, pack_words, nullptr, 0u);
      MIRGE_LAUNCH_CHECK(ctx, "trim_kernel(pass 1)");
    }
    unsigned grid2 = split ? grid / 4 + 1 : grid / 16 + 1;
    if (grid2 > (unsigned)ctx->sm_count * (split ? 64u : 8u)) grid2 = (unsigned)ctx->sm_count * (split ? 64u : 8u);
    trim_kernel<32, true, 2, false><<<grid2, TRIM_THREADS, extra, stream>>>(d_fastq, nbytes, d_line_start, n_records, win, d_key_off,
                                                                          d_keys, keys_capacity_words, ctrl, 0u, d_slow, so, il, pack_words, nullptr, 0u);
  } else if (ctx->max_adapter_len <= 32) {
    MIRGE_CUDA(ctx, cudaFuncSetAttribute(trim_kernel<32, false, 0, false>, cudaFuncAttributeMaxDynamicSharedMemorySize, 96 * 1024));
    trim_kernel<32, false, 0, false><<<grid, TRIM_THREADS, smem, stream>>>(d_fastq, nbytes, d_line_start, n_records, win, d_key_off,
                                                                           d_keys, keys_capacity_words, ctrl, smem, nullptr, so, il, 8, nullptr, 0u);
  } else {
    MIRGE_CUDA(ctx, cudaFuncSetAttribute(trim_kernel<64, false, 0, false>, cudaFuncAttributeMaxDynamicSharedMemorySize, 96 * 1024));
    trim_kernel<64, false, 0, false><<<grid, TRIM_THREADS, smem, stream>>>(d_fastq, nbytes, d_line_start, n_records, win, d_key_off,
                                                                           d_keys, keys_capacity_words, ctrl, smem, nullptr, so, il, 8, nullptr, 0u);
  }
  MIRGE_LAUNCH_CHECK(ctx, "trim_kernel");
  return MIRGE_OK;
}

static uint64_t dt_tiles(uint64_t nbytes) { return (nbytes + 16) / DT_TILE + 1; }
static uint64_t dt_slow_cap(uint64_t n_cap) { return n_cap; }

extern "C" int mirge_digest_fused_ok(const mirge_ctx *ctx) {
  if (!ctx || !ctx->params_set) return 0;
  return ctx->fast_ok && ctx->split_ok && ctx->trim_mode == 0;
}

extern "C" uint64_t mirge_digest_scratch_bytes(uint64_t nbytes, uint64_t n_cap) {
  const uint64_t n = n_cap ? n_cap : 1;
  return align16(8 * dt_tiles(nbytes)) + align16(sizeof(SlowRec) * dt_slow_cap(n)) + align16(4 * n) + align16(sizeof(DpEntry) * n) +
         align16(4ull * MAX_PACK_WORDS * n) + 64;
}

extern "C" int mirge_digest_tiles(mirge_ctx *ctx, const uint8_t *d_fastq, uint64_t nbytes, int is_final, uint64_t n_cap,
                                  uint32_t *d_line_start, uint16_t *d_win, uint32_t *d_key_off, uint32_t *d_keys,
                                  uint64_t keys_capacity_words, uint64_t *d_trim_ctrl, void *d_scratch, uint64_t *d_ins,
                                  uint64_t ins_capacity, void *stream_) {
  if (!ctx) return MIRGE_ERR_ARG;
  if (!ctx->params_set) MIRGE_FAIL(ctx, MIRGE_ERR_ARG, "digest: mirge_set_trim_params has not been called");
  if (!mirge_digest_fused_ok(ctx)) MIRGE_FAIL(ctx, MIRGE_ERR_ARG, "digest: the fused path needs 3' adapters of <= 32 nt with indels (use mirge_trim)");
  if (nbytes == 0) return MIRGE_OK;
  if (!d_fastq || !d_keys || !d_trim_ctrl || !d_scratch || n_cap == 0) MIRGE_FAIL(ctx, MIRGE_ERR_ARG, "digest: null buffer");
  if (nbytes > 0xFFFFFF00ull) MIRGE_FAIL(ctx, MIRGE_ERR_ARG, "digest: batch larger than 4 GiB - 256");
  if (!d_win != !d_key_off) MIRGE_FAIL(ctx, MIRGE_ERR_ARG, "digest: d_win and d_key_off go together");
  if (!d_key_off && !d_ins) MIRGE_FAIL(ctx, MIRGE_ERR_ARG, "digest: neither per-slot outputs nor an insert list requested");
  if (d_ins && (ins_capacity < n_cap * (uint64_t)trim_slots_of(&ctx->params) || ((uintptr_t)d_ins & 7)))
    MIRGE_FAIL(ctx, MIRGE_ERR_ARG, "digest: bad insert list");
  if (((uintptr_t)d_line_start & 15) || ((uintptr_t)d_win & 7) || ((uintptr_t)d_scratch & 15)) MIRGE_FAIL(ctx, MIRGE_ERR_ARG, "digest: misaligned buffer");
  if (n_cap >= 0x80000000ull || n_cap * (uint64_t)trim_slots_of(&ctx->params) >= MAX_LIST_ITEMS)
    MIRGE_FAIL(ctx, MIRGE_ERR_ARG, "digest: more than 2^28 emission slots in one batch (use smaller batches)");
  cudaStream_t stream = (cudaStream_t)stream_;
  MIRGE_CUDA(ctx, cudaSetDevice(ctx->device));
  const uint32_t skew = (uint32_t)((uintptr_t)d_fastq & 15);
  DigestTilesArgs A;
  A.fq = d_fastq - skew;
  A.n = nbytes + skew;
  A.skew = skew;
  A.is_final = is_final ? 1u : 0u;
  A.n_tiles = A.n / DT_TILE + 1;
  uint8_t *sc = (uint8_t *)d_scratch;
  A.tile_state = (unsigned long long *)sc;
  sc += align16(8 * dt_tiles(nbytes));
  A.ss.r_list = nullptr;
  A.ss.recs = (SlowRec *)sc;
  A.ss.cap = dt_slow_cap(n_cap);
  sc += align16(sizeof(SlowRec) * A.ss.cap);
  uint32_t *d_redo = (uint32_t *)sc;
  sc += align16(4 * n_cap);
  A.so.entries = (DpEntry *)sc;
  sc += align16(sizeof(DpEntry) * n_cap);
  A.so.pk = (uint32_t *)sc;
  A.so.cap = n_cap;
  A.line_start = d_line_start;
  A.n_cap = (uint32_t)n_cap;
  A.win = (ushort4 *)d_win;
  A.key_off = d_key_off;
  A.keys = d_keys;
  A.keys_cap = keys_capacity_words;
  A.ctrl = (unsigned long long *)d_trim_ctrl;
  A.il = InsList{(uint2 *)d_ins, d_ins ? ins_capacity : 0};
  const uint64_t avg = (nbytes + n_cap - 1) / n_cap;
  A.pack_words = avg <= 2 * 112 + 40 ? 8 : MAX_PACK_WORDS;
  MIRGE_CUDA(ctx, cudaMemsetAsync(A.tile_state, 0, 8 * A.n_tiles, stream));
  const size_t rows = (size_t)PS_ROWS_OF(A.pack_words) * TRIM_THREADS * 4;
  const size_t dt_smem = (size_t)DT_NBUF * DT_LOAD + (size_t)DT_NBUF * DT_WORDS * 4 + (size_t)DT_NBUF * (DT_WORDS + 2) * 2 +
                         (size_t)ctx->params.n_adapters * 1024 + DT_GROUPS * rows;
  MIRGE_CUDA(ctx, cudaFuncSetAttribute(digest_tiles_kernel, cudaFuncAttributeMaxDynamicSharedMemorySize, 200 * 1024));
  int per_sm = 0;
  MIRGE_CUDA(ctx, cudaOccupancyMaxActiveBlocksPerMultiprocessor(&per_sm, digest_tiles_kernel, DT_THREADS, dt_smem));
  if (per_sm < 1) MIRGE_FAIL(ctx, MIRGE_ERR_CUDA, "digest: the fused kernel does not fit an SM");
  uint64_t grid = (uint64_t)ctx->sm_count * per_sm;
  if (grid > A.n_tiles) grid = A.n_tiles;
  digest_tiles_kernel<<<(unsigned)grid, DT_THREADS, dt_smem, stream>>>(A);
  MIRGE_LAUNCH_CHECK(ctx, "digest_tiles_kernel");
  const unsigned lgrid = (unsigned)((n_cap + TRIM_THREADS - 1) / TRIM_THREADS);
  const size_t extra = (size_t)ctx->params.n_adapters * 1024 + rows;
  const size_t dp_smem = extra + (size_t)TRIM_THREADS * (sizeof(DpEntry) + 4 + 2);
  trim_dp_kernel<true><<<lgrid, TRIM_THREADS, dp_smem, stream>>>(A.so.entries, A.so.pk, A.so.cap, d_redo, A.win, d_key_off, d_keys,
                                                                 keys_capacity_words, A.ctrl, A.il, A.pack_words);
  MIRGE_LAUNCH_CHECK(ctx, "trim_dp_kernel(stage 2)");
  trim_dp_kernel<false><<<lgrid, TRIM_THREADS, dp_smem, stream>>>(A.so.entries, A.so.pk, A.so.cap, d_redo, A.win, d_key_off, d_keys,
                                                                  keys_capacity_words, A.ctrl, A.il, A.pack_words);
  MIRGE_LAUNCH_CHECK(ctx, "trim_dp_kernel(stage 3)");
  unsigned grid2 = lgrid / 4 + 1;
  if (grid2 > (unsigned)ctx->sm_count * 64u) grid2 = (unsigned)ctx->sm_count * 64u;
  trim_kernel<32, true, 2, false><<<grid2, TRIM_THREADS, extra, stream>>>(A.fq, A.n, d_line_start, n_cap, A.win, d_key_off, d_keys,
                                                                        keys_capacity_words, A.ctrl, 0u, nullptr, A.so, A.il,
                                                                        A.pack_words, A.ss.recs, (uint32_t)n_cap);
  MIRGE_LAUNCH_CHECK(ctx, "trim_kernel(whole-pipeline pass)");
  return MIRGE_OK;
}

extern "C" int mirge_trim_mode(mirge_ctx *ctx, int mode) {
  if (!ctx || mode < 0 || mode > 2) return MIRGE_ERR_ARG;
  ctx->trim_mode = mode;
  return MIRGE_OK;
}
```

Before: 1234.

## Resume deferred DP reads from saved state and move per-read scratch to shared memory

The DP trimming kernel now saves the Myers search state (bit vectors, queue, best match, loop position) into a per-entry resume record when stage 2 defers a read. Stage 3 can then continue from that point instead of rescanning the read from the start. Per-thread slot arrays and the traceback column buffer move from local memory to shared memory. The kernels become grid-stride loops launched through a helper. The intent is to cut redundant recomputation and local-memory spills, at the cost of extra global scratch, more shared memory per block that may lower occupancy, and a more complex control flow.

New measurement: 1206, median of 6. -2.2%, worse.

```diff
diff --git a/mirge3.0_b200/csrc/adapter_search.cuh b/mirge3.0_b200/csrc/adapter_search.cuh
--- a/mirge3.0_b200/csrc/adapter_search.cuh
+++ b/mirge3.0_b200/csrc/adapter_search.cuh
@@ -267,6 +267,7 @@
   const uint32_t *ps;
   bool jump_ok;
   int rbase;
+  uint32_t *cols;
 };
 
 struct ByteRead {
@@ -309,8 +310,25 @@
 };
 
 struct ColBuf {
-  uint32_t vp[RB], vn[RB];
+  uint32_t vp_[RB], vn_[RB];
   int j0;
+  using Ref = ColBuf &;
+  __device__ __forceinline__ void bind(const FastCtx &) {}
+  __device__ __forceinline__ uint32_t vp(int t) const { return vp_[t]; }
+  __device__ __forceinline__ uint32_t vn(int t) const { return vn_[t]; }
+  __device__ __forceinline__ void set(int t, uint32_t vp, uint32_t vn) { vp_[t] = vp; vn_[t] = vn; }
+};
+struct SharedColBuf {
+  uint32_t *p;
+  int j0;
+  using Ref = SharedColBuf;
+  __device__ __forceinline__ void bind(const FastCtx &fc) { p = fc.cols; }
+  __device__ __forceinline__ uint32_t vp(int t) const { return p[2 * t * TRIM_THREADS]; }
+  __device__ __forceinline__ uint32_t vn(int t) const { return p[(2 * t + 1) * TRIM_THREADS]; }
+  __device__ __forceinline__ void set(int t, uint32_t vp, uint32_t vn) {
+    p[2 * t * TRIM_THREADS] = vp;
+    p[(2 * t + 1) * TRIM_THREADS] = vn;
+  }
 };
 
 __device__ __forceinline__ int cell_cost(uint32_t vp, uint32_t vn, int r) {
@@ -332,20 +350,16 @@
     (vn) = hp_ & xv_;                                             \
   }
 
-template <class RV>
-__device__ __noinline__ void recompute(const uint32_t *eqt, const RV read, int jc, int span, ColBuf &cb) {
-  const int j0 = max(0, jc - span);
+template <class RV, class CBR>
+__device__ __noinline__ void recompute(const uint32_t *eqt, const RV read, int jc, CBR cb) {
   uint32_t vp = 0xFFFFFFFFu, vn = 0u;
-  cb.j0 = j0;
-  cb.vp[0] = vp;
-  cb.vn[0] = vn;
+  cb.set(0, vp, vn);
   int t = 1;
-  for (int j = j0 + 1; j <= jc; ++j, ++t) {
+  for (int j = cb.j0 + 1; j <= jc; ++j, ++t) {
     const uint32_t eq = read.eq(eqt, j - 1);
     uint32_t hp, hn;
     MYERS_STEP(eq, vp, vn, hp, hn)
-    cb.vp[t] = vp;
-    cb.vn[t] = vn;
+    cb.set(t, vp, vn);
   }
 }
 
@@ -356,9 +370,10 @@
   return ((uint64_t)hi << 32) | lo;
 }
 
-template <class RV>
-__device__ __noinline__ void traceback(const int a, const uint32_t *eqt, const RV read, const FastCtx &fc, const ColBuf &cb,
-                                          int i, int j, int c, int &matches, int &origin) {
+struct TraceOut { int matches, origin; };
+template <class RV, class CBR>
+__device__ __noinline__ TraceOut traceback(const int a, const uint32_t *eqt, const RV read, const FastCtx fc, const CBR cb,
+                                           int i, int j, int c) {
   const bool jump = fc.jump_ok && !c_p.ad[a].wildcard_ref;
   const uint64_t a2 = c_p.ad[a].a2;
   int r = i, col = j, cost = c, nonmatch = 0;
@@ -386,14 +401,13 @@
       continue;
     }
     const int t0 = col - cb.j0;
-    const uint32_t vp0 = cb.vp[t0], vn0 = cb.vn[t0], vp1 = cb.vp[t0 - 1], vn1 = cb.vn[t0 - 1];
+    const uint32_t vp0 = cb.vp(t0), vn0 = cb.vn(t0), vp1 = cb.vp(t0 - 1), vn1 = cb.vn(t0 - 1);
     const int cd = cell_cost(vp1, vn1, r - 1) + 1, cdel = cell_cost(vp1, vn1, r) + 1, cins = cell_cost(vp0, vn0, r - 1) + 1;
     if (cd <= cdel && cd <= cins) { --r; --col; ++nonmatch; cost = cd - 1; }
     else if (cins <= cdel) { --r; ++nonmatch; cost = cins - 1; }
     else { --col; cost = cdel - 1; }
   }
-  origin = col - r;
-  matches = i - nonmatch;
+  return TraceOut{i - nonmatch, col - r};
 }
 
 __device__ __forceinline__ bool traceback_cost1(const int a, const FastCtx &fc, int i, int j, int &matches, int &origin) {
@@ -447,8 +461,15 @@
 #define INS_MASK(eq, vp, hn) (~(eq) & (vp) & ((hn) << 1))
 #define CHAIN_LEN(ins, i) (__clz((int)~((ins) << (32 - (i)))))
 
-template <bool DEFER, class RV>
-__device__ __forceinline__ int locate_fast(const int a, const RV read, const int n, const FastCtx &fc, Match &out) {
+struct FastResume {
+  uint32_t st;
+  uint32_t vp, vn, hp, hn, eq;
+  uint32_t q0, q1, q2, q3;
+  uint32_t bo;
+};
+template <bool DEFER, class RV, class CB = ColBuf>
+__device__ __forceinline__ int locate_fast(const int a, const RV read, const int n, const FastCtx &fc, Match &out,
+                                           FastResume *rs = nullptr) {
   const unsigned lanes = __activemask();
   const DevAdapter &ad = c_p.ad[a];
   const int m = ad.m;
@@ -460,8 +481,9 @@
   int score = m;
   bool have = false;
   int b_m = 0, b_c = 0, b_o = 0, b_idx = 0;
-  bool stopped = false;
-  ColBuf cb;
+  bool stopped = false, in_tail = false;
+  CB cb;
+  cb.bind(fc);
   uint32_t q0 = 0, q1 = 0, q2 = 0, q3 = 0;
   bool pend = false, pend_ins = false, need_slow = false;
   uint32_t pend_v = 0;
@@ -475,7 +497,6 @@
     if (q2 && (!v_ || Q_COST(q2) < Q_COST(v_))) { v_ = q2; which_ = 2; }                         \
     if (q3 && (!v_ || Q_COST(q3) < Q_COST(v_))) { v_ = q3; which_ = 3; }                         \
     if (which_ < 0) break;                                                                       \
-    if (which_ == 0) q0 = 0; else if (which_ == 1) q1 = 0; else if (which_ == 2) q2 = 0; else q3 = 0; \
     const int jc_ = Q_COL(v_), cc_ = Q_COST(v_), t_ = Q_CHAIN(v_);                               \
     const int ir_ = m - t_, cr_ = cc_ - t_;           \
     int ub_ = t_ ? ir_ : Q_UB(v_, m);                                                            \
@@ -486,16 +507,27 @@
         mt_ = ir_; org_ = jc_ - ir_;                                                             \
       } else if (!(cr_ == 1 && traceback_cost1(a, fc, ir_, jc_, mt_, org_))) {                   \
         if (DEFER) { need_slow = true; break; }                                                  \
-        recompute(eqt, read, jc_, span, cb);                                                     \
-        traceback(a, eqt, read, fc, cb, ir_, jc_, cr_, mt_, org_);                               \
+        cb.j0 = max(0, jc_ - span);                                                              \
+        recompute<RV, typename CB::Ref>(eqt, read, jc_, cb);                                     \
+        const TraceOut to_ = traceback<RV, typename CB::Ref>(a, eqt, read, fc, cb, ir_, jc_, cr_); \
+        mt_ = to_.matches; org_ = to_.origin;                                                    \
       }                                                                                          \
       TAKE_IF_BETTER(mt_, cc_, org_, jc_)                                                        \
     }                                                                                            \
+    if (which_ == 0) q0 = 0; else if (which_ == 1) q1 = 0; else if (which_ == 2) q2 = 0; else q3 = 0; \
   }
 
   uint32_t hp = 0, hn = 0;
+  const bool resume = !DEFER && rs && (rs->st & 1u);
+  if (resume) {
+    const FastResume s = *rs;
+    have = (s.st >> 1) & 1u; b_m = (int)((s.st >> 8) & 0xFFu); b_c = (int)((s.st >> 16) & 0xFFu);
+    b_o = (int)(s.bo & 0xFFFFu); b_idx = (int)(s.bo >> 16);
+    vp = s.vp; vn = s.vn; hp = s.hp; hn = s.hn; eq = s.eq;
+    q0 = s.q0; q1 = s.q1; q2 = s.q2; q3 = s.q3;
+  }
   auto cur = read.cursor();
-  for (int j = 1; j <= n; ++j) {
+  for (int j = 1; j <= (resume ? 0 : n); ++j) {
     eq = cur.next(eqt);
     MYERS_STEP(eq, vp, vn, hp, hn)
     score += (hp & top) ? 1 : 0;
@@ -541,6 +573,7 @@
   __syncwarp(lanes);
   const unsigned scan_lanes = __ballot_sync(lanes, !stopped && !need_slow);
   if (!stopped && !need_slow) {
+    in_tail = true;
     uint32_t rowmask = 0, rowub = 0;
     const uint32_t hps = hp << 1, hns = hn << 1;
     const uint32_t ins = n >= 1 ? INS_MASK(eq, vp, hn) : 0u;
@@ -583,16 +616,31 @@
         } else if (!(cr == 1 && traceback_cost1(a, fc, ir, n, mt, org))) {
           if (DEFER) { need_slow = true; break; }
           if (!have_cols) {
-            recompute(eqt, read, n, span, cb);
+            cb.j0 = max(0, n - span);
+            recompute<RV, typename CB::Ref>(eqt, read, n, cb);
             have_cols = true;
           }
-          traceback(a, eqt, read, fc, cb, ir, n, cr, mt, org);
+          const TraceOut to = traceback<RV, typename CB::Ref>(a, eqt, read, fc, cb, ir, n, cr);
+          mt = to.matches;
+          org = to.origin;
         }
         TAKE_IF_BETTER(mt, ci, org, idx)
       }
     }
   }
-  if (DEFER && need_slow) return 2;
+  if (DEFER && need_slow) {
+    if (rs && in_tail) {
+      FastResume s;
+      s.st = 1u | (have ? 2u : 0u) | ((uint32_t)b_m << 8) | ((uint32_t)b_c << 16);
+      s.vp = vp; s.vn = vn; s.hp = hp; s.hn = hn; s.eq = eq;
+      s.q0 = q0; s.q1 = q1; s.q2 = q2; s.q3 = q3;
+      s.bo = (uint32_t)b_o | ((uint32_t)b_idx << 16);
+      *rs = s;
+    } else if (rs) {
+      rs->st = 0u;
+    }
+    return 2;
+  }
   if (!have) return 0;
   out.rstart = b_o;
   out.rstop = b_idx <= n ? b_idx : n;
diff --git a/mirge3.0_b200/csrc/trim.cu b/mirge3.0_b200/csrc/trim.cu
--- a/mirge3.0_b200/csrc/trim.cu
+++ b/mirge3.0_b200/csrc/trim.cu
@@ -873,11 +873,23 @@
   flush_stats(ctrl);
 }
 
+struct DpResume {
+  uint32_t pos;
+  uint32_t t;
+  uint32_t se;
+  uint32_t best;
+  FastResume fast;
+  uint32_t pad;
+};
+static_assert(sizeof(DpResume) == 64, "DpResume is four 16-byte words");
+
+#define DP_SLOT_STRIDE(E) ((E) | 1)
+
 template <bool FIRST>
 __global__ void __launch_bounds__(TRIM_THREADS, FIRST ? 7 : 4)
 trim_dp_kernel(const DpEntry *__restrict__ entries, const uint32_t *__restrict__ pk, uint64_t cap, uint32_t *__restrict__ redo,
-               ushort4 *__restrict__ win, uint32_t *__restrict__ key_off, uint32_t *__restrict__ keys, uint64_t keys_cap,
-               unsigned long long *__restrict__ ctrl, const InsList il, const int pack_words) {
+               DpResume *__restrict__ rsm, ushort4 *__restrict__ win, uint32_t *__restrict__ key_off, uint32_t *__restrict__ keys,
+               uint64_t keys_cap, unsigned long long *__restrict__ ctrl, const InsList il, const int pack_words) {
   extern __shared__ uint4 smem4[];
   uint32_t *eq = (uint32_t *)smem4;
   uint32_t *ps_base = eq + c_p.n_adapters * 256;
@@ -885,121 +897,182 @@
   uint32_t *s_hist = (uint32_t *)(s_ent + TRIM_THREADS);
   uint16_t *s_order = (uint16_t *)(s_hist + TRIM_THREADS);
   const int tid = threadIdx.x, lane = tid & 31;
+  const int E = c_p.slots, n_mods = c_p.n_mods, ws = DP_SLOT_STRIDE(E);
+  uint32_t *s_slots = (uint32_t *)(s_order + TRIM_THREADS);
+  int *w_start = (int *)s_slots + tid * ws, *w_stop = (int *)s_slots + (TRIM_THREADS + tid) * ws;
+  uint32_t *w_words = s_slots + (2 * TRIM_THREADS + tid) * ws;
+  const int *w_zero = (const int *)s_slots + 3 * TRIM_THREADS * ws;
+  uint32_t *cols = s_slots + (3 * TRIM_THREADS + 1) * ws + tid;
   const unsigned long long n_items = FIRST ? ctrl[6] : ctrl[7];
-  const uint64_t base = (uint64_t)blockIdx.x * TRIM_THREADS;
-  if (base >= n_items) return;
+  if ((uint64_t)blockIdx.x * TRIM_THREADS >= n_items) return;
   init_stats(pack_words);
   for (int e = tid; e < c_p.n_adapters * 4; e += TRIM_THREADS) eq[(e >> 2) * 256 + (e & 3)] = (uint32_t)c_p.ad[e >> 2].peq[e & 3];
-  const int n_here = (int)min((unsigned long long)TRIM_THREADS, n_items - base);
-  uint32_t my_e = 0;
-  int bin = TRIM_THREADS - 1;
-  if (tid < n_here) {
-    my_e = FIRST ? (uint32_t)(base + tid) : redo[base + tid];
-    const uint4 v = *(const uint4 *)(entries + my_e);
-    DpEntry de = *(const DpEntry *)&v;
-    de.pad = my_e;
-    s_ent[tid] = de;
-    const int wl = (int)(de.se >> 16) - (int)(de.se & 0xFFFFu);
-    bin = TRIM_THREADS - 1 - min(wl, TRIM_THREADS - 1);
-  }
-  s_hist[tid] = 0;
-  __syncthreads();
-  if (tid < n_here) atomicAdd(&s_hist[bin], 1u);
-  __syncthreads();
-  if (tid < 32) {
-    uint32_t h[TRIM_THREADS / 32], sum = 0;
+  for (int s = tid; s < ws; s += TRIM_THREADS) ((int *)w_zero)[s] = 0;
+  for (uint64_t base = (uint64_t)blockIdx.x * TRIM_THREADS; base < n_items; base += (uint64_t)gridDim.x * TRIM_THREADS) {
+    const int n_here = (int)min((unsigned long long)TRIM_THREADS, n_items - base);
+    int bin = TRIM_THREADS - 1;
+    if (tid < n_here) {
+      const uint32_t my_e = FIRST ? (uint32_t)(base + tid) : redo[base + tid];
+      const uint4 v = *(const uint4 *)(entries + my_e);
+      DpEntry de = *(const DpEntry *)&v;
+      de.pad = my_e;
+      s_ent[tid] = de;
+      const int wl = (int)(de.se >> 16) - (int)(de.se & 0xFFFFu);
+      bin = TRIM_THREADS - 1 - min(wl, TRIM_THREADS - 1);
+    }
+    s_hist[tid] = 0;
+    __syncthreads();
+    if (tid < n_here) atomicAdd(&s_hist[bin], 1u);
+    __syncthreads();
+    if (tid < 32) {
+      uint32_t h[TRIM_THREADS / 32], sum = 0;
 #pragma unroll
-    for (int q = 0; q < TRIM_THREADS / 32; ++q) { h[q] = s_hist[(TRIM_THREADS / 32) * tid + q]; sum += h[q]; }
-    uint32_t incl = sum;
+      for (int q = 0; q < TRIM_THREADS / 32; ++q) { h[q] = s_hist[(TRIM_THREADS / 32) * tid + q]; sum += h[q]; }
+      uint32_t incl = sum;
 #pragma unroll
-    for (int d = 1; d < 32; d <<= 1) {
-      const uint32_t x = __shfl_up_sync(0xffffffffu, incl, d);
-      if (lane >= d) incl += x;
-    }
-    uint32_t run = incl - sum;
+      for (int d = 1; d < 32; d <<= 1) {
+        const uint32_t x = __shfl_up_sync(0xffffffffu, incl, d);
+        if (lane >= d) incl += x;
+      }
+      uint32_t run = incl - sum;
 #pragma unroll
-    for (int q = 0; q < TRIM_THREADS / 32; ++q) { s_hist[(TRIM_THREADS / 32) * tid + q] = run; run += h[q]; }
-  }
-  __syncthreads();
-  if (tid < n_here) s_order[atomicAdd(&s_hist[bin], 1u)] = (uint16_t)tid;
-  __syncthreads();
-  const bool valid = tid < n_here;
-  const int E = c_p.slots, n_mods = c_p.n_mods;
-  const bool qia = false;
-  int w_start[MIRGE_MAX_MODS], w_stop[MIRGE_MAX_MODS], w_us[MIRGE_MAX_MODS], w_ue[MIRGE_MAX_MODS];
-  uint32_t w_words[MIRGE_MAX_MODS];
-#pragma unroll 1
-  for (int s = 0; s < E; ++s) { w_start[s] = w_stop[s] = w_us[s] = w_ue[s] = 0; w_words[s] = 0; }
-  uint32_t *ps_mine = ps_base + tid;
-  const int mi_ad = first_adapter_mod();
-  uint64_t r = 0;
-  bool need_redo = false;
-  int slot_lo = (E == 1) ? 0 : mi_ad, slot_hi = E;
-  uint32_t ent_id = 0;
-  if (valid) {
-    const DpEntry de = s_ent[s_order[tid]];
-    r = de.r;
-    ent_id = de.pad;
-    int start = (int)(de.se & 0xFFFFu), stop = (int)(de.se >> 16);
-    const int nwords = ((int)de.sl + 15) >> 4;
-#pragma unroll 1
-    for (int w = 0; w < PS_ROWS_OF(pack_words); ++w) {
-      if (w < nwords) cp_async_4(ps_mine + w * TRIM_THREADS, pk + (uint64_t)w * cap + ent_id);
-      else ps_mine[w * TRIM_THREADS] = 0u;
-    }
-    cp_async_wait_all();
-    FastCtx fc;
-    fc.s_eq = eq; fc.ps = ps_mine; fc.jump_ok = true; fc.rbase = 0;
-#pragma unroll 1
-    for (int mi = mi_ad; mi < n_mods && !need_redo; ++mi) {
-      const int kind = c_p.kind[mi];
-      if (kind == MIRGE_MOD_ADAPTER) {
-#pragma unroll 1
-        for (int t = 0; t < c_p.times; ++t) {
-          fc.rbase = start;
-          const PackedRead rv{ps_mine, start};
-          const int n = stop - start;
-          Match best;
-          int which = -1;
-#pragma unroll 1
-          for (int a = 0; a < c_p.n_adapters; ++a) {
-            Match mt;
-            const int rc = locate_fast<FIRST>(a, rv, n, fc, mt);
-            if (rc == 2) { need_redo = true; break; }
-            if (rc == 0) continue;
-            if (which < 0 || mt.matches > best.matches || (mt.matches == best.matches && mt.errors < best.errors)) { best = mt; which = a; }
+      for (int q = 0; q < TRIM_THREADS / 32; ++q) { s_hist[(TRIM_THREADS / 32) * tid + q] = run; run += h[q]; }
+    }
+    __syncthreads();
+    if (tid < n_here) s_order[atomicAdd(&s_hist[bin], 1u)] = (uint16_t)tid;
+    __syncthreads();
+    const bool valid = tid < n_here;
+    const bool qia = false;
+#pragma unroll 1
+    for (int s = 0; s < E; ++s) { w_start[s] = w_stop[s] = 0; w_words[s] = 0; }
+    uint32_t *ps_mine = ps_base + tid;
+    const int mi_ad = first_adapter_mod();
+    uint64_t r = 0;
+    bool need_redo = false;
+    int slot_lo = (E == 1) ? 0 : mi_ad, slot_hi = E;
+    uint32_t ent_id = 0;
+    if (valid) {
+      const DpEntry de = s_ent[s_order[tid]];
+      r = de.r;
+      ent_id = de.pad;
+      int start = (int)(de.se & 0xFFFFu), stop = (int)(de.se >> 16);
+      const int nwords = ((int)de.sl + 15) >> 4;
+#pragma unroll 1
+      for (int w = 0; w < PS_ROWS_OF(pack_words); ++w) {
+        if (w < nwords) cp_async_4(ps_mine + w * TRIM_THREADS, pk + (uint64_t)w * cap + ent_id);
+        else ps_mine[w * TRIM_THREADS] = 0u;
+      }
+      FastCtx fc;
+      fc.s_eq = eq; fc.ps = ps_mine; fc.jump_ok = true; fc.rbase = 0; fc.cols = cols;
+      DpResume *const rec = rsm + ent_id;
+      int mi = mi_ad, t0 = 0, a0 = 0, which = -1;
+      Match best{0, 0, 0, 0};
+      FastResume *resume = nullptr;
+      if (!FIRST) {
+        const uint4 h = *(const uint4 *)rec;
+        mi = (int)(h.x & 0xFFu); a0 = (int)((h.x >> 8) & 0xFFu); which = (int)((h.x >> 16) & 0xFFu) - 1;
+        t0 = (int)h.y;
+        start = (int)(h.z & 0xFFFFu); stop = (int)(h.z >> 16);
+        best.rstart = (int)(h.w & 0xFFFFu); best.matches = (int)((h.w >> 16) & 0xFFu); best.errors = (int)(h.w >> 24);
+        resume = &rec->fast;
+      }
+      cp_async_wait_all();
+#pragma unroll 1
+      for (; mi < n_mods && !need_redo; ++mi) {
+        const int kind = c_p.kind[mi];
+        if (kind == MIRGE_MOD_ADAPTER) {
+#pragma unroll 1
+          for (int t = t0; t < c_p.times; ++t) {
+            fc.rbase = start;
+            const PackedRead rv{ps_mine, start};
+            const int n = stop - start;
+#pragma unroll 1
+            for (int a = a0; a < c_p.n_adapters; ++a) {
+              Match mt;
+              int rc;
+              if (FIRST) {
+                rc = locate_fast<true>(a, rv, n, fc, mt, &rec->fast);
+              } else {
+                rc = locate_fast<false, PackedRead, SharedColBuf>(a, rv, n, fc, mt, resume);
+                resume = nullptr;
+              }
+              if (rc == 2) {
+                need_redo = true;
+                if (E != 1 && mi > mi_ad) {
+                  *(uint4 *)rec = make_uint4((uint32_t)mi_ad, 0u, de.se, 0u);
+                  rec->fast.st = 0u;
+                } else {
+                  const uint32_t bw = (uint32_t)best.rstart | ((uint32_t)best.matches << 16) | ((uint32_t)best.errors << 24);
+                  *(uint4 *)rec = make_uint4((uint32_t)mi | ((uint32_t)a << 8) | ((uint32_t)(which + 1) << 16), (uint32_t)t,
+                                             (uint32_t)start | ((uint32_t)stop << 16), bw);
+                }
+                break;
+              }
+              if (rc == 0) continue;
+              if (which < 0 || mt.matches > best.matches || (mt.matches == best.matches && mt.errors < best.errors)) { best = mt; which = a; }
+            }
+            a0 = 0;
+            if (need_redo || which < 0) break;
+            stop = start + best.rstart;
+            which = -1;
           }
-          if (need_redo || which < 0) break;
-          stop = start + best.rstart;
-        }
-      } else if (kind == MIRGE_MOD_CUT) {
-        const int c = c_p.a[mi], len = stop - start;
-        if (c > 0) start += min(c, len);
-        else stop = start + max(len + c, 0);
-      }
-      if (!need_redo) { RECORD_SLOT(mi) }
-    }
-  }
-  if (FIRST) {
-    const unsigned rm = __ballot_sync(0xffffffffu, need_redo);
-    if (rm) {
-      const int leader = __ffs(rm) - 1;
-      unsigned long long b2 = 0;
-      if (lane == leader) b2 = atomicAdd(ctrl + 7, (unsigned long long)__popc(rm));
-      b2 = __shfl_sync(0xffffffffu, b2, leader);
-      if (need_redo) redo[b2 + __popc(rm & ((1u << lane) - 1u))] = ent_id;
-    }
-    if (need_redo) slot_hi = slot_lo;
-  }
-  emit_record<true, 0>(valid, r, E, slot_lo, slot_hi, nullptr, true, w_start, w_stop, w_us, w_ue, w_words, false, win, key_off, keys, keys_cap,
-                       ctrl, SlowSink{nullptr, nullptr, 0}, make_uint4(0, 0, 0, 0), 0u, ps_mine, il);
+          t0 = 0;
+          which = -1;
+        } else if (kind == MIRGE_MOD_CUT) {
+          const int c = c_p.a[mi], len = stop - start;
+          if (c > 0) start += min(c, len);
+          else stop = start + max(len + c, 0);
+        }
+        if (!need_redo) { RECORD_SLOT(mi) }
+      }
+    }
+    if (FIRST) {
+      const unsigned rm = __ballot_sync(0xffffffffu, need_redo);
+      if (rm) {
+        const int leader = __ffs(rm) - 1;
+        unsigned long long b2 = 0;
+        if (lane == leader) b2 = atomicAdd(ctrl + 7, (unsigned long long)__popc(rm));
+        b2 = __shfl_sync(0xffffffffu, b2, leader);
+        if (need_redo) redo[b2 + __popc(rm & ((1u << lane) - 1u))] = ent_id;
+      }
+      if (need_redo) slot_hi = slot_lo;
+    }
+    emit_record<true, 0>(valid, r, E, slot_lo, slot_hi, nullptr, true, w_start, w_stop, w_zero, w_zero, w_words, false, win, key_off, keys,
+                         keys_cap, ctrl, SlowSink{nullptr, nullptr, 0}, make_uint4(0, 0, 0, 0), 0u, ps_mine, il);
+    __syncthreads();
+  }
   flush_stats(ctrl);
+}
+
+template <bool FIRST>
+static int launch_dp(mirge_ctx *ctx, const SplitOut so, uint32_t *redo, DpResume *rsm, ushort4 *win, uint32_t *key_off, uint32_t *keys,
+                     uint64_t keys_cap, unsigned long long *ctrl, const InsList il, int pack_words, uint64_t max_items,
+                     cudaStream_t stream) {
+  const mirge_trim_params &p = ctx->params;
+  size_t smem = (size_t)p.n_adapters * 1024 + (size_t)PS_ROWS_OF(pack_words) * TRIM_THREADS * 4 +
+                (size_t)TRIM_THREADS * (sizeof(DpEntry) + 4 + 2) + (size_t)(3 * TRIM_THREADS + 1) * DP_SLOT_STRIDE(trim_slots_of(&p)) * 4;
+  if (!FIRST) {
+    int cols = 0;
+    for (int a = 0; a < p.n_adapters; ++a) cols = max(cols, p.adapters[a].m + 2 * p.adapters[a].k + 3);
+    smem += (size_t)2 * cols * TRIM_THREADS * 4;
+  }
+  MIRGE_CUDA(ctx, cudaFuncSetAttribute(trim_dp_kernel<FIRST>, cudaFuncAttributeMaxDynamicSharedMemorySize, (int)smem));
+  int per_sm = 0;
+  MIRGE_CUDA(ctx, cudaOccupancyMaxActiveBlocksPerMultiprocessor(&per_sm, trim_dp_kernel<FIRST>, TRIM_THREADS, smem));
+  if (per_sm < 1) MIRGE_FAIL(ctx, MIRGE_ERR_CUDA, "trim: the DP kernel does not fit an SM");
+  uint64_t grid = (uint64_t)ctx->sm_count * per_sm;
+  const uint64_t chunks = (max_items + TRIM_THREADS - 1) / TRIM_THREADS;
+  if (grid > chunks) grid = chunks;
+  trim_dp_kernel<FIRST><<<(unsigned)grid, TRIM_THREADS, smem, stream>>>(so.entries, so.pk, so.cap, redo, rsm, win, key_off, keys, keys_cap,
+                                                                        ctrl, il, pack_words);
+  MIRGE_LAUNCH_CHECK(ctx, FIRST ? "trim_dp_kernel(stage 2)" : "trim_dp_kernel(stage 3)");
+  return MIRGE_OK;
 }
 
 static uint64_t align16(uint64_t x) { return (x + 15) & ~15ull; }
 extern "C" uint64_t mirge_trim_scratch_bytes(uint64_t n_records) {
   const uint64_t n = n_records ? n_records : 1;
-  return 2 * align16(4 * n) + align16(sizeof(DpEntry) * n) + align16(4ull * MAX_PACK_WORDS * n) + 64;
+  return 2 * align16(4 * n) + align16(sizeof(DpEntry) * n) + align16(4ull * MAX_PACK_WORDS * n) + sizeof(DpResume) * n + 64;
 }
 
 extern "C" int mirge_trim(mirge_ctx *ctx, const uint8_t *d_fastq, uint64_t nbytes, const uint32_t *d_line_start, uint64_t n_records,
@@ -1046,6 +1119,7 @@
     so.entries = (DpEntry *)(sc + 2 * align16(4 * n_records));
     so.pk = (uint32_t *)(sc + 2 * align16(4 * n_records) + align16(sizeof(DpEntry) * n_records));
     so.cap = n_records;
+    DpResume *rsm = (DpResume *)((uint8_t *)so.pk + align16(4ull * MAX_PACK_WORDS * n_records));
     const int pack_words = avg <= 2 * 112 + 40 ? 8 : MAX_PACK_WORDS;
     const size_t extra = (size_t)ctx->params.n_adapters * 1024 + (size_t)PS_ROWS_OF(pack_words) * TRIM_THREADS * 4;
     if (split) {
@@ -1053,13 +1127,10 @@
       trim_kernel<32, true, 1, true><<<grid, TRIM_THREADS, smem + extra, stream>>>(d_fastq, nbytes, d_line_start, n_records, win, d_key_off,
                                                                                  d_keys, keys_capacity_words, ctrl, smem, d_slow, so, il, pack_words, nullptr, 0u);
       MIRGE_LAUNCH_CHECK(ctx, "trim_kernel(stage 1)");
-      const size_t dp_smem = extra + (size_t)TRIM_THREADS * (sizeof(DpEntry) + 4 + 2);
-      trim_dp_kernel<true><<<grid, TRIM_THREADS, dp_smem, stream>>>(so.entries, so.pk, so.cap, d_redo, win, d_key_off, d_keys,
-                                                                    keys_capacity_words, ctrl, il, pack_words);
-      MIRGE_LAUNCH_CHECK(ctx, "trim_dp_kernel(stage 2)");
-      trim_dp_kernel<false><<<grid, TRIM_THREADS, dp_smem, stream>>>(so.entries, so.pk, so.cap, d_redo, win, d_key_off, d_keys,
-                                                                     keys_capacity_words, ctrl, il, pack_words);
-      MIRGE_LAUNCH_CHECK(ctx, "trim_dp_kernel(stage 3)");
+      int rc = launch_dp<true>(ctx, so, d_redo, rsm, win, d_key_off, d_keys, keys_capacity_words, ctrl, il, pack_words, n_records, stream);
+      if (rc == MIRGE_OK)
+        rc = launch_dp<false>(ctx, so, d_redo, rsm, win, d_key_off, d_keys, keys_capacity_words, ctrl, il, pack_words, n_records, stream);
+      if (rc != MIRGE_OK) return rc;
     } else {
       MIRGE_CUDA(ctx, cudaFuncSetAttribute(trim_kernel<32, true, 1, false>, cudaFuncAttributeMaxDynamicSharedMemorySize, 200 * 1024));
       trim_kernel<32, true, 1, false><<<grid, TRIM_THREADS, smem + extra, stream>>>(d_fastq, nbytes, d_line_start, n_records, win,
@@ -1095,7 +1166,7 @@
 extern "C" uint64_t mirge_digest_scratch_bytes(uint64_t nbytes, uint64_t n_cap) {
   const uint64_t n = n_cap ? n_cap : 1;
   return align16(8 * dt_tiles(nbytes)) + align16(sizeof(SlowRec) * dt_slow_cap(n)) + align16(4 * n) + align16(sizeof(DpEntry) * n) +
-         align16(4ull * MAX_PACK_WORDS * n) + 64;
+         align16(4ull * MAX_PACK_WORDS * n) + sizeof(DpResume) * n + 64;
 }
 
 extern "C" int mirge_digest_tiles(mirge_ctx *ctx, const uint8_t *d_fastq, uint64_t nbytes, int is_final, uint64_t n_cap,
@@ -1137,6 +1208,8 @@
   sc += align16(sizeof(DpEntry) * n_cap);
   A.so.pk = (uint32_t *)sc;
   A.so.cap = n_cap;
+  sc += align16(4ull * MAX_PACK_WORDS * n_cap);
+  DpResume *rsm = (DpResume *)sc;
   A.line_start = d_line_start;
   A.n_cap = (uint32_t)n_cap;
   A.win = (ushort4 *)d_win;
@@ -1161,13 +1234,10 @@
   MIRGE_LAUNCH_CHECK(ctx, "digest_tiles_kernel");
   const unsigned lgrid = (unsigned)((n_cap + TRIM_THREADS - 1) / TRIM_THREADS);
   const size_t extra = (size_t)ctx->params.n_adapters * 1024 + rows;
-  const size_t dp_smem = extra + (size_t)TRIM_THREADS * (sizeof(DpEntry) + 4 + 2);
-  trim_dp_kernel<true><<<lgrid, TRIM_THREADS, dp_smem, stream>>>(A.so.entries, A.so.pk, A.so.cap, d_redo, A.win, d_key_off, d_keys,
-                                                                 keys_capacity_words, A.ctrl, A.il, A.pack_words);
-  MIRGE_LAUNCH_CHECK(ctx, "trim_dp_kernel(stage 2)");
-  trim_dp_kernel<false><<<lgrid, TRIM_THREADS, dp_smem, stream>>>(A.so.entries, A.so.pk, A.so.cap, d_redo, A.win, d_key_off, d_keys,
-                                                                  keys_capacity_words, A.ctrl, A.il, A.pack_words);
-  MIRGE_LAUNCH_CHECK(ctx, "trim_dp_kernel(stage 3)");
+  int rc = launch_dp<true>(ctx, A.so, d_redo, rsm, A.win, d_key_off, d_keys, keys_capacity_words, A.ctrl, A.il, A.pack_words, n_cap, stream);
+  if (rc == MIRGE_OK)
+    rc = launch_dp<false>(ctx, A.so, d_redo, rsm, A.win, d_key_off, d_keys, keys_capacity_words, A.ctrl, A.il, A.pack_words, n_cap, stream);
+  if (rc != MIRGE_OK) return rc;
   unsigned grid2 = lgrid / 4 + 1;
   if (grid2 > (unsigned)ctx->sm_count * 64u) grid2 = (unsigned)ctx->sm_count * 64u;
   trim_kernel<32, true, 2, false><<<grid2, TRIM_THREADS, extra, stream>>>(A.fq, A.n, d_line_start, n_cap, A.win, d_key_off, d_keys,
diff --git a/profiles/trim_stages_time.py b/profiles/trim_stages_time.py
--- /dev/null
+++ b/profiles/trim_stages_time.py
@@ -0,0 +1,127 @@
+import argparse
+import importlib.util
+import json
+import os
+import statistics
+import subprocess
+import sys
+
+sys.dont_write_bytecode = True
+HERE = os.path.dirname(os.path.abspath(__file__))
+
+STAGES = {
+    "trim_kernel<32, true, 1, true>": "stage1",
+    "trim_dp_kernel<true>": "stage2",
+    "trim_dp_kernel<false>": "stage3",
+    "trim_kernel<32, true, 2, false>": "whole_pipeline",
+}
+
+
+def card():
+    import torch
+
+    name = torch.cuda.get_device_name(0)
+    try:
+        q = subprocess.run(["nvidia-smi", "--query-gpu=power.limit", "--format=csv,noheader", "-i", "0"], capture_output=True,
+                           text=True, timeout=30)
+        power = q.stdout.strip() or "unknown"
+    except (OSError, subprocess.SubprocessError):
+        power = "unknown"
+    return name, power
+
+
+def stage_of(kernel_name):
+    base = kernel_name.split("(", 1)[0]
+    if base.startswith("void "):
+        base = base[5:]
+    return STAGES.get(base.strip())
+
+
+def summary(xs):
+    return {"best": round(min(xs), 3), "median": round(statistics.median(xs), 3), "all": [round(x, 3) for x in xs]}
+
+
+def main():
+    ap = argparse.ArgumentParser()
+    ap.add_argument("--tree", default=os.path.dirname(HERE), help="checkout whose mirge_b200 is timed")
+    ap.add_argument("--reads", type=int, default=50_000_000)
+    ap.add_argument("--mrna", type=int, default=100_000, help="mRNA entries of the libraries the reads are drawn from (C2: 100 k)")
+    ap.add_argument("--batch-mb", type=int, default=2048)
+    ap.add_argument("--steps", type=int, default=7)
+    ap.add_argument("--warmup", type=int, default=2)
+    ap.add_argument("--prof-steps", type=int, default=2)
+    a = ap.parse_args()
+    if a.steps < 1 or a.prof_steps < 1:
+        raise SystemExit("trim_stages_time: --steps and --prof-steps must be >= 1")
+    tree = os.path.abspath(a.tree)
+    sys.path.insert(0, tree)
+    import torch
+
+    import mirge_b200
+    from mirge_b200 import device as D
+    from mirge_b200 import synth
+
+    spec = importlib.util.spec_from_file_location("bench_for_sample", os.path.join(os.path.dirname(HERE), "bench.py"))
+    bench = importlib.util.module_from_spec(spec)
+    spec.loader.exec_module(bench)
+
+    dev = D.Device(0)
+    torch.cuda.set_device(dev.tdev)
+    libs = synth.make_libraries(mrna_count=a.mrna)
+    cfg = synth.trim_config_for(2, "head")
+    eng = D.DigestEngine(dev, cfg)
+    fq = bench.sample_fastq(libs, 2, 0, a.reads, False, dev.tdev)
+    table = D.CollapseTable(dev, min_keys=1 << 22)
+    batch_bytes = a.batch_mb << 20
+    torch.cuda.synchronize()
+
+    def one_pass():
+        table.reset()
+        return eng.digest_device(fq, table, batch_bytes)
+
+    for _ in range(a.warmup):
+        one_pass()
+    torch.cuda.synchronize()
+    dp0, redo0 = eng.stats.get("dp_reads", 0), eng.stats.get("dp_redo", 0)
+    dev.timing = True
+    dev.timer_totals(reset=True)
+    pass_ms, trim_ms, n = [], [], 0
+    for _ in range(a.steps):
+        st = torch.cuda.current_stream(dev.tdev)
+        e0, e1 = torch.cuda.Event(enable_timing=True), torch.cuda.Event(enable_timing=True)
+        e0.record(st)
+        n = one_pass()
+        e1.record(st)
+        torch.cuda.synchronize()
+        pass_ms.append(e0.elapsed_time(e1))
+        trim_ms.append(dev.timer_totals(reset=True).get("trim", (0, 0.0))[1])
+    dev.timing = False
+    dp_frac = (eng.stats.get("dp_reads", 0) - dp0) / max(n * a.steps, 1)
+    redo_frac = (eng.stats.get("dp_redo", 0) - redo0) / max(n * a.steps, 1)
+
+    from torch.profiler import ProfilerActivity, profile
+
+    with profile(activities=[ProfilerActivity.CUDA]) as prof:
+        for _ in range(a.prof_steps):
+            one_pass()
+        torch.cuda.synchronize()
+    stages = {k: 0.0 for k in STAGES.values()}
+    launches = {k: 0 for k in STAGES.values()}
+    for ev in prof.events():
+        s = stage_of(ev.name)
+        if s is None or getattr(ev, "device_type", None) != torch.autograd.DeviceType.CUDA:
+            continue
+        stages[s] += ev.time_range.elapsed_us() / 1000.0
+        launches[s] += 1
+    name, power = card()
+    print(json.dumps({
+        "tree": tree, "device": name, "power_limit": power, "reads": n, "batch_mb": a.batch_mb,
+        "steps": a.steps, "warmup": a.warmup, "pass_ms": summary(pass_ms), "trim_ms": summary(trim_ms),
+        "stages_ms_per_pass": {k: round(v / a.prof_steps, 3) for k, v in stages.items()},
+        "stage_launches_per_pass": {k: v / a.prof_steps for k, v in launches.items()},
+        "dp_search_frac": round(dp_frac, 4), "cost_column_frac": round(redo_frac, 4),
+    }), flush=True)
+
+
+if __name__ == "__main__":
+    main()
```
